# leighghunt/kart

Measured on AMD Instinct MI355X. Metric: feature deltas classified+field-diffed/sec (M/s) at 1/2/4/8 GPUs; % HBM peak, higher is better.
Workload: dtype u8/u64 (integer + fp64 compare); 1 GPU; C3: ONE 100000000-polygon int-PK layer, 10% edits (4% geometry + 4% attribute updates, 1% del, 1% ins), two-commit diff + field diff; features=100000000, delta_order=walk (= key) order, then pk order (kd_delta_pk_order), side_order=git tree (walk) order as listed, no side sort, parallelism=bucket-range shards x1

## Files before the change

### kart_amd/csrc/kd_classify.hip

```cpp
#include <cstdlib>

#include "kd_join.h"

namespace kd {

#ifndef KD_RS3_PROBE_NOSEARCH
#define KD_RS3_PROBE_NOSEARCH 0
#endif
#ifndef KD_RS3_PROBE_NOOID
#define KD_RS3_PROBE_NOOID 0
#endif
#ifndef KD_RS3_PROBE_NONAMES
#define KD_RS3_PROBE_NONAMES 0
#endif
constexpr int C3_NT = 256;
constexpr int C3_CH = 1024;
#ifndef KD_C3_SAMPLE_BITS
#define KD_C3_SAMPLE_BITS 11
#endif
constexpr int C3_SAMPLE_BITS = KD_C3_SAMPLE_BITS;
constexpr int C3_SAMPLES = 1 << C3_SAMPLE_BITS;

struct Resolve3Args {
    const u64 *A, *O, *T;
// ... 232 lines not shown
        if (tid == 0) {
            if (tclean) atomicAdd((unsigned long long*)g.counts, (unsigned long long)tclean);
            if (base + cnt == n) {
                g.counts[1] = exc + tc;
                g.counts[2] = exm + tm;
            }
        }
        u64 pc = exc + (off & 0xFFFF), pm = exm + (off >> 16);
#pragma unroll
        for (int j = 0; j < PT; j++) {
            if (cls[j] == 2) {
                u32* o = g.out_conf + 3 * pc;
                o[0] = ia[j]; o[1] = io[j]; o[2] = itt[j];
                pc++;
            } else if (cls[j] == 1) {
                g.out_md[pm] = rec[j];
                pm++;
            }
        }
    }
}

}

using namespace kd;

int kd::resolve3_have_a(kd_ctx* ctx, const kd_side& A, const kd_side& O, const kd_side& T, const u32* cand3,
                        const u64* c2, u32* d_conf, uint2* d_md, u64* counts, u32* derr, const u32* pA, const u32* pO,
                        const u32* pT) {
    const bool perm = pA || pO || pT;
    int rc;
    const u64 nA = A.n, nO = O.n, nT = T.n;
    const u64 nchunk = (nO + nT) / C3_CH + 2;
    void *desc, *aux, *dz;
    if ((rc = ensure(ctx, "c3.desc", 2 * nchunk * 8, &desc))) return rc;
    const bool fresh_aux = ctx->bufs["c3.aux"].p == nullptr;
    if ((rc = ensure(ctx, "c3.aux", 64, &aux))) return rc;
    if (fresh_aux) KD_HIP(hipMemsetAsync(aux, 0, 64, ctx->stream));
    if ((rc = device_zeros(ctx, &dz))) return rc;
    rc = launch(ctx, "k_sorted3", [&] {
        const u64 blocks = std::min<u64>((2 * nchunk + 255) / 256, (u64)ctx->n_cu * 8);
        hipLaunchKernelGGL(k_sorted3, dim3((unsigned)std::max<u64>(blocks, 1)), dim3(256), 0, ctx->stream,
                           (const u64*)dz, (u64)0, (u64*)desc, 2 * nchunk, (u32*)aux, counts);
    });
    if (rc) return rc;
    const int occ_r3a = occupancy(ctx, perm ? (const void*)k_resolve3<C3_NT, true, true> : (const void*)k_resolve3<C3_NT, false, true>,
                                  C3_NT, 0);
    auto ptr = [&](const void* p, u64 n) { return n && p ? p : (const void*)dz; };
    Resolve3Args g{};
    g.A = (const u64*)dz; g.O = (const u64*)ptr(O.key, nO); g.T = (const u64*)ptr(T.key, nT);
    g.oA = (const u32*)ptr(A.oid, nA); g.oO = (const u32*)ptr(O.oid, nO); g.oT = (const u32*)ptr(T.oid, nT);
    g.nA = nA; g.nO = nO;
    g.nmA = (const u8*)ptr(A.name, nA); g.nmO = (const u8*)ptr(O.name, nO); g.nmT = (const u8*)ptr(T.name, nT);
    g.noA = (const u64*)ptr(A.name_off, nA); g.noO = (const u64*)ptr(O.name_off, nO); g.noT = (const u64*)ptr(T.name_off, nT);
    g.hash_mode = A.key_mode == KD_KEY_HASH;
    g.cand = nullptr; g.cand3 = cand3; g.c2 = c2;
    g.pA = (const u32*)ptr(pA, nA); g.pO = (const u32*)ptr(pO, nO); g.pT = (const u32*)ptr(pT, nT);
    g.desc = (u64*)desc; g.nchunk = nchunk; g.aux = (u32*)aux;
    g.out_conf = d_conf; g.out_md = d_md; g.counts = counts; g.err = derr;
    const u64 grid = std::min<u64>((nO + nT) / C3_CH + 1, (u64)ctx->n_cu * (u64)occ_r3a);
    return launch(ctx, "k_resolve3", [&] {
        if (perm) hipLaunchKernelGGL((k_resolve3<C3_NT, true, true>), dim3((unsigned)grid), dim3(C3_NT), 0, ctx->stream, g);
        else hipLaunchKernelGGL((k_resolve3<C3_NT, false, true>), dim3((unsigned)grid), dim3(C3_NT), 0, ctx->stream, g);
    });
}

int kd::stage_side(kd_ctx* ctx, const kd_side* s, const char* tag, kd_side* dev) {
    *dev = *s;
    dev->mem = KD_MEM_DEVICE;
    std::string p(tag);
    int rc;
    if ((rc = stage_in(ctx, (p + ".key").c_str(), s->key, s->n * 8, s->mem, (const void**)&dev->key))) return rc;
    if ((rc = stage_in(ctx, (p + ".oid").c_str(), s->oid, s->n * 20, s->mem, (const void**)&dev->oid))) return rc;
    if (s->key_mode == KD_KEY_HASH && s->n) {
        KD_CHECK(s->name_off && s->name, "KD_KEY_HASH side without filenames");
        u64 nbytes = s->mem == KD_MEM_HOST ? s->name_off[s->n] : 0;
        if (s->mem == KD_MEM_DEVICE) {
            KD_HIP(hipMemcpy(&nbytes, s->name_off + s->n, 8, hipMemcpyDeviceToHost));
        }
        if ((rc = stage_in(ctx, (p + ".noff").c_str(), s->name_off, (s->n + 1) * 8, s->mem, (const void**)&dev->name_off))) return rc;
        if ((rc = stage_in(ctx, (p + ".name").c_str(), s->name, nbytes ? nbytes : 1, s->mem, (const void**)&dev->name))) return rc;
    }
    return KD_OK;
}

int kd::check_side(const kd_side* s, const char* which) {
    KD_CHECK(s, "%s side is NULL", which);
    KD_CHECK(s->n == 0 || (s->key && s->oid), "%s side: key/oid NULL", which);
    KD_CHECK(s->mem == KD_MEM_HOST || s->mem == KD_MEM_DEVICE, "%s side: bad mem", which);
    KD_CHECK(s->key_mode == KD_KEY_INT || s->key_mode == KD_KEY_HASH, "%s side: bad key_mode", which);
    return KD_OK;
}

static int merge3_device(kd_ctx* ctx, const kd_side& A, const kd_side& O, const kd_side& T, u32* d_conf, uint2* d_md,
                         u64* counts, u32* derr, const u32* pA = nullptr, const u32* pO = nullptr,
                         const u32* pT = nullptr) {
    const bool perm = pA || pO || pT;
    int rc;
    const u64 nA = A.n, nO = O.n, nT = T.n;
    if (nO + nT > 0 && ctx->opt.merge3_join)
        return merge3_join_device(ctx, A, O, T, d_conf, d_md, counts, derr, pA, pO, pT);
    const u64 nchunk = (nO + nT) / C3_CH + 2;
    void *cand, *c2, *desc, *aux, *dz;
    if ((rc = ensure(ctx, "c3.cand", (nO + nT + 1) * 8, &cand))) return rc;
    if ((rc = ensure(ctx, "c3.c2", 64, &c2))) return rc;
    if ((rc = ensure(ctx, "c3.desc", 2 * nchunk * 8, &desc))) return rc;
    const bool fresh_aux = ctx->bufs["c3.aux"].p == nullptr;
    if ((rc = ensure(ctx, "c3.aux", 64, &aux))) return rc;
    if (fresh_aux) KD_HIP(hipMemsetAsync(aux, 0, 64, ctx->stream));
    if ((rc = device_zeros(ctx, &dz))) return rc;
    const u64* kA = nA ? A.key : (const u64*)dz;
    rc = launch(ctx, "k_sorted3", [&] {
        const u64 work = std::max<u64>(nA / 2, 2 * nchunk);
        const u64 blocks = std::min<u64>((work + 255) / 256, (u64)ctx->n_cu * 8);
        hipLaunchKernelGGL(k_sorted3, dim3((unsigned)std::max<u64>(blocks, 1)), dim3(256), 0, ctx->stream, kA, nA,
                           (u64*)desc, 2 * nchunk, (u32*)aux, counts);
    });
    if (rc) return rc;
    if ((rc = diff2_device(ctx, &O, &T, 0, (u32*)cand, nullptr, (u64*)c2, derr, perm ? pO : nullptr,
                           perm ? pT : nullptr)))
        return rc;
    ctx->occ_resolve3 = occupancy(ctx, perm ? (const void*)k_resolve3<C3_NT, true, false> : (const void*)k_resolve3<C3_NT, false, false>,
                                  C3_NT, 0);
    auto ptr = [&](const void* p, u64 n) { return n && p ? p : (const void*)dz; };
    Resolve3Args g;
    g.A = kA; g.O = (const u64*)ptr(O.key, nO); g.T = (const u64*)ptr(T.key, nT);
    g.oA = (const u32*)ptr(A.oid, nA); g.oO = (const u32*)ptr(O.oid, nO); g.oT = (const u32*)ptr(T.oid, nT);
    g.nA = nA; g.nO = nO;
    g.nmA = (const u8*)ptr(A.name, nA); g.nmO = (const u8*)ptr(O.name, nO); g.nmT = (const u8*)ptr(T.name, nT);
    g.noA = (const u64*)ptr(A.name_off, nA); g.noO = (const u64*)ptr(O.name_off, nO); g.noT = (const u64*)ptr(T.name_off, nT);
    g.hash_mode = A.key_mode == KD_KEY_HASH;
    g.cand = (const uint2*)cand; g.c2 = (const u64*)c2;
    g.pA = (const u32*)ptr(pA, nA); g.pO = (const u32*)ptr(pO, nO); g.pT = (const u32*)ptr(pT, nT);
    g.desc = (u64*)desc; g.nchunk = nchunk; g.aux = (u32*)aux;
    g.out_conf = d_conf; g.out_md = d_md; g.counts = counts; g.err = derr;
    const u64 grid = std::min<u64>((nO + nT) / C3_CH + 1, (u64)ctx->n_cu * (u64)ctx->occ_resolve3);
    return launch(ctx, "k_resolve3", [&] {
        if (perm) hipLaunchKernelGGL((k_resolve3<C3_NT, true, false>), dim3((unsigned)grid), dim3(C3_NT), 0, ctx->stream, g);
        else hipLaunchKernelGGL((k_resolve3<C3_NT, false, false>), dim3((unsigned)grid), dim3(C3_NT), 0, ctx->stream, g);
    });
}

extern "C" {

int kd_reserve(kd_ctx* ctx, uint64_t max_entries_per_side, uint64_t max_updates) {
    KD_CHECK(ctx, "kd_reserve: ctx NULL");
    KD_HIP(hipSetDevice(ctx->device));
    u64 total = 2 * max_entries_per_side;
    u64 ntiles = (total + C2_TILE - 1) / C2_TILE + 1;
    void* p;
    int rc;
    if ((rc = ensure(ctx, "c2.part", (ntiles + 1) * 8, &p))) return rc;
    if ((rc = ensure(ctx, "c2.tcnt", ntiles * 16, &p))) return rc;
    if ((rc = ensure(ctx, "c2.gsum", 2 * (ntiles / 64 + 1) * 8, &p))) return rc;
    if ((rc = ensure(ctx, "c2.sdel", ntiles * (C2_TILE + 64) * 8, &p))) return rc;
    (void)max_updates;
    return KD_OK;
}

int kd_diff2_device(kd_ctx* ctx, const kd_side* base, const kd_side* target, uint32_t flags, uint32_t* d_delta,
                    uint32_t* d_upd, uint64_t* d_counts, uint32_t* d_err) {
    KD_CHECK(ctx, "kd_diff2_device: ctx NULL");
    int rc;
    if ((rc = check_side(base, "base")) || (rc = check_side(target, "target"))) return rc;
    KD_CHECK(base->mem == KD_MEM_DEVICE && target->mem == KD_MEM_DEVICE, "kd_diff2_device: sides must be device memory");
    KD_CHECK(d_delta && d_counts && d_err, "kd_diff2_device: NULL output");
    KD_HIP(hipSetDevice(ctx->device));
    return diff2_device(ctx, base, target, flags, d_delta, d_upd, d_counts, d_err);
}

int kd_diff2_device_perm(kd_ctx* ctx, const kd_side* base, const kd_side* target, const uint32_t* base_order,
                         const uint32_t* target_order, uint32_t flags, uint32_t* d_delta, uint32_t* d_upd,
                         uint64_t* d_counts, uint32_t* d_err) {
    KD_CHECK(ctx, "kd_diff2_device_perm: ctx NULL");
    int rc;
    if ((rc = check_side(base, "base")) || (rc = check_side(target, "target"))) return rc;
    KD_CHECK(base->mem == KD_MEM_DEVICE && target->mem == KD_MEM_DEVICE, "kd_diff2_device_perm: sides must be device memory");
    KD_CHECK(d_delta && d_counts && d_err, "kd_diff2_device_perm: NULL output");
    KD_CHECK((base->n == 0 || base_order) && (target->n == 0 || target_order), "kd_diff2_device_perm: NULL order");
    KD_HIP(hipSetDevice(ctx->device));
    return diff2_device(ctx, base, target, flags, d_delta, d_upd, d_counts, d_err,
                        base_order ? base_order : (const u32*)nullptr, target_order);
}

int kd_diff2_device_ex(kd_ctx* ctx, const kd_side* base, const kd_side* target, const uint32_t* base_order,
                       const uint32_t* target_order, uint32_t flags, uint32_t* d_delta, uint32_t* d_upd,
                       uint64_t* d_delta_key, uint64_t* d_upd_key, uint64_t* d_counts, uint32_t* d_err) {
    KD_CHECK(ctx, "kd_diff2_device_ex: ctx NULL");
    int rc;
    if ((rc = check_side(base, "base")) || (rc = check_side(target, "target"))) return rc;
    KD_CHECK(base->mem == KD_MEM_DEVICE && target->mem == KD_MEM_DEVICE, "kd_diff2_device_ex: sides must be device memory");
    KD_CHECK(d_delta && d_counts && d_err, "kd_diff2_device_ex: NULL output");
    KD_CHECK(!base_order == !target_order, "kd_diff2_device_ex: both orders or neither");
    KD_CHECK(!d_upd_key || (d_upd && d_delta_key), "kd_diff2_device_ex: update keys need the update list and delta keys");
    KD_HIP(hipSetDevice(ctx->device));
    void* dz = nullptr;
    if (base_order && (rc = device_zeros(ctx, &dz))) return rc;
    const u32* oa = base_order ? (base->n ? base_order : (const u32*)dz) : nullptr;
    const u32* ob = target_order ? (target->n ? target_order : (const u32*)dz) : nullptr;
    return diff2_device(ctx, base, target, flags, d_delta, d_upd, d_counts, d_err, oa, ob, d_delta_key, d_upd_key);
}

int kd_diff2_step(kd_ctx* ctx, const kd_step* s) {
    KD_CHECK(ctx && s, "kd_diff2_step: NULL");
    int rc;
    if ((rc = check_side(s->base, "base")) || (rc = check_side(s->target, "target"))) return rc;
    KD_CHECK(s->base->mem == KD_MEM_DEVICE && s->target->mem == KD_MEM_DEVICE, "kd_diff2_step: sides must be device memory");
    KD_CHECK(s->d_delta && s->d_counts && s->d_err, "kd_diff2_step: NULL output");
    KD_CHECK(!s->base_order == !s->target_order, "kd_diff2_step: both orders or neither");
    KD_CHECK(!s->d_upd_key || (s->d_upd && s->d_delta_key), "kd_diff2_step: update keys need the update list and delta keys");
    const bool have_fd = s->old_blobs != nullptr;
    KD_CHECK(!have_fd || (s->new_blobs && s->maps && s->d_masks && s->d_status), "kd_diff2_step: field diff: NULL argument");
    const bool have_dpk = s->d_delta_pk != nullptr, have_upk = s->d_upd_pk != nullptr;
    KD_CHECK(!have_dpk || s->d_delta_perm, "kd_diff2_step: d_delta_pk without d_delta_perm");
    KD_CHECK(!have_upk || (s->d_upd_perm && s->d_upd), "kd_diff2_step: d_upd_pk needs d_upd_perm and the update list");
    KD_HIP(hipSetDevice(ctx->device));
    void* dz = nullptr;
    if ((rc = device_zeros(ctx, &dz))) return rc;
    const u32* oa = s->base_order ? (s->base->n ? s->base_order : (const u32*)dz) : nullptr;
    const u32* ob = s->target_order ? (s->target->n ? s->target_order : (const u32*)dz) : nullptr;
    Diff2Place pl;
    if ((rc = diff2_front(ctx, s->base, s->target, s->flags, s->d_delta, s->d_upd, s->d_counts, s->d_err, oa, ob,
                          s->d_delta_key, s->d_upd_key, &pl)))
        return rc;
    const int ov = ctx->opt.step_overlap;
    auto field_diff = [&]() -> int {
        return have_fd ? kd_fielddiff(ctx, s->old_blobs, s->new_blobs, s->d_pairs, s->upd_cap, s->d_counts + 1,
                                      KD_MEM_DEVICE, s->maps, s->d_masks, s->d_status, KD_MEM_DEVICE)
                       : KD_OK;
    };
    auto pk_orders = [&](bool lds_free) -> int {
        int r = KD_OK;
        if (have_dpk)
            r = delta_pk_order(ctx, s->base, s->target, s->d_delta, s->d_delta_key, s->delta_cap, s->d_counts + 3,
                               s->pk_lo, s->pk_hi, s->d_delta_pk, s->d_delta_perm, lds_free);
        if (!r && have_upk)
            r = delta_pk_order(ctx, s->base, s->target, s->d_upd, s->d_upd_key, s->upd_cap, s->d_counts + 1, s->pk_lo,
                               s->pk_hi, s->d_upd_pk, s->d_upd_perm, lds_free);
        return r;
    };
    const bool place_aside = !(have_fd && s->d_pairs);
    const bool overlap = ov > 0 && have_fd && pl.needed && (place_aside || have_dpk || have_upk) &&
                         s->base->n + s->target->n >= ctx->opt.step_overlap_min;
    const int wave = ctx->opt.pkm_wave;
    if (!overlap) {
        if ((rc = diff2_place(ctx, pl)) || (rc = field_diff())) return rc;
        return pk_orders(wave > 0);
    }
    if (!ctx->side_stream) {
        KD_HIP(hipStreamCreateWithFlags(&ctx->side_stream, hipStreamNonBlocking));
        KD_HIP(hipEventCreateWithFlags(&ctx->ev_fork, hipEventDisableTiming));
        KD_HIP(hipEventCreateWithFlags(&ctx->ev_join, hipEventDisableTiming));
    }
    const hipStream_t main = ctx->stream, side = ctx->side_stream;
    if (!place_aside && (rc = diff2_place(ctx, pl))) return rc;
    KD_HIP(hipEventRecord(ctx->ev_fork, main));
    auto side_work = [&]() -> int {
        StreamScope scope(ctx, side);
        KD_HIP(hipStreamWaitEvent(side, ctx->ev_fork, 0));
        int r = place_aside ? diff2_place(ctx, pl) : KD_OK;
        return r ? r : pk_orders(wave != 0);
    };
    int rc_fd, rc_side = KD_OK;
    if (ov == 2) {
        rc_side = side_work();
        rc_fd = field_diff();
    } else {
        rc_fd = field_diff();
        if (!rc_fd) rc_side = side_work();
    }
    hipError_t e = hipEventRecord(ctx->ev_join, side);
    if (e == hipSuccess) e = hipStreamWaitEvent(main, ctx->ev_join, 0);
    if (e != hipSuccess) {
        const hipError_t e2 = hipStreamSynchronize(side);
        if (!rc_fd && !rc_side) {
            set_error("kd_diff2_step: join: %s", hipGetErrorString(e2 != hipSuccess ? e2 : e));
            return KD_EHIP;
        }
    }
    return rc_fd ? rc_fd : rc_side;
}

int kd_diff2(kd_ctx* ctx, const kd_side* base, const kd_side* target, uint32_t flags, kd_diff_result** out) {
    KD_CHECK(ctx && out, "kd_diff2: NULL");
    int rc;
    if ((rc = check_side(base, "base")) || (rc = check_side(target, "target"))) return rc;
    KD_HIP(hipSetDevice(ctx->device));
    host_mark(ctx, nullptr);
    kd_side A, B;
    if ((rc = stage_side(ctx, base, "in.a", &A)) || (rc = stage_side(ctx, target, "in.b", &B))) return rc;
    host_mark(ctx, "kd_diff2 stage");
    u64 total = base->n + target->n;
    void *dd, *du, *dc;
    if ((rc = ensure(ctx, "out.delta", (total + 1) * 8, &dd))) return rc;
    if ((rc = ensure(ctx, "out.upd", (total + 1) * 8, &du))) return rc;
    if ((rc = ensure(ctx, "out.counts", 64, &dc))) return rc;
    host_mark(ctx, "kd_diff2 ensure");
    u64* counts = (u64*)dc;
    u32* derr = (u32*)(counts + 4);
    if ((rc = diff2_device(ctx, &A, &B, flags, (u32*)dd, (u32*)du, counts, derr))) return rc;
    host_mark(ctx, "kd_diff2 kernels");
    u64 hc[5];
    KD_HIP(hipMemcpyAsync(hc, dc, 40, hipMemcpyDeviceToHost, ctx->stream));
    KD_HIP(hipStreamSynchronize(ctx->stream));
    u32 err = (u32)(hc[4] & 0xFFFFFFFFu);
    if (err) {
        set_error("kd_diff2: %s", (err & 1) ? "side keys not strictly ascending" : "hash key collision between different filenames");
        return KD_EUNSUPPORTED;
    }
    u64 nd = hc[3], nu = hc[1];
    host_mark(ctx, "kd_diff2 counts");
    size_t bytes = sizeof(kd_diff_result) + (nd + nu) * 8 + 16;
    kd_diff_result* r = (kd_diff_result*)std::malloc(bytes);
    KD_CHECK(r, "kd_diff2: out of host memory");
    host_mark(ctx, "kd_diff2 malloc");
    r->n_insert = hc[0]; r->n_update = hc[1]; r->n_delete = hc[2]; r->n_delta = nd;
    r->delta = (u32*)(r + 1);
    r->upd = r->delta + 2 * nd;
    if (nd) {
        if ((rc = stage_d2h(ctx, r->delta, dd, nd * 8)) || (nu && (rc = stage_d2h(ctx, r->upd, du, nu * 8)))) {
            std::free(r);
            return rc;
        }
    }
    host_mark(ctx, "kd_diff2 results");
    prof_flush(ctx);
    *out = r;
    return KD_OK;
}

int kd_merge3(kd_ctx* ctx, const kd_side* anc, const kd_side* ours, const kd_side* theirs, uint32_t flags,
              kd_merge_result** out) {
    (void)flags;
    KD_CHECK(ctx && out, "kd_merge3: NULL");
    int rc;
    if ((rc = check_side(anc, "ancestor")) || (rc = check_side(ours, "ours")) || (rc = check_side(theirs, "theirs"))) return rc;
    KD_CHECK(anc->key_mode == ours->key_mode && ours->key_mode == theirs->key_mode, "kd_merge3: key modes differ");
    KD_CHECK(anc->n < 0xFFFFFFFFull && ours->n < 0xFFFFFFFFull && theirs->n < 0xFFFFFFFFull, "kd_merge3: side too large");
    KD_HIP(hipSetDevice(ctx->device));
    kd_side A, O, T;
    if ((rc = stage_side(ctx, anc, "in.a", &A)) || (rc = stage_side(ctx, ours, "in.b", &O)) ||
        (rc = stage_side(ctx, theirs, "in.c", &T)))
        return rc;
    const u64 nA = A.n, nO = O.n, nT = T.n;
    void *oc, *om, *dc;
    if ((rc = ensure(ctx, "c3.oc", (nA + nO + nT + 1) * 12, &oc))) return rc;
    if ((rc = ensure(ctx, "c3.om", (nO + nT + 1) * 8, &om))) return rc;
    if ((rc = ensure(ctx, "c3.counts", 64, &dc))) return rc;
    u64* counts = (u64*)dc;
    u32* derr = (u32*)(counts + 4);
    if ((rc = merge3_device(ctx, A, O, T, (u32*)oc, (uint2*)om, counts, derr))) return rc;
    u64 hc[5];
    KD_HIP(hipMemcpyAsync(hc, dc, 40, hipMemcpyDeviceToHost, ctx->stream));
    KD_HIP(hipStreamSynchronize(ctx->stream));
    u32 err = (u32)(hc[4] & 0xFFFFFFFFu);
    if (err) {
        set_error("kd_merge3: err=0x%x (%s)", err,
                  (err & 1) ? "keys not strictly ascending" : (err & 2) ? "hash key collision" : "tile overflow");
        return KD_EUNSUPPORTED;
    }
    u64 nc = hc[1], nm = hc[2];
    kd_merge_result* r = (kd_merge_result*)std::malloc(sizeof(kd_merge_result) + nc * 12 + nm * 8 + 16);
    KD_CHECK(r, "kd_merge3: out of host memory");
    r->n_clean = hc[0]; r->n_conflict = nc; r->n_mdelta = nm;
    r->conflict = (u32*)(r + 1);
    r->mdelta = r->conflict + 3 * nc;
    if ((nc && (rc = stage_d2h(ctx, r->conflict, oc, nc * 12))) || (nm && (rc = stage_d2h(ctx, r->mdelta, om, nm * 8)))) {
        std::free(r);
        return rc;
    }
    prof_flush(ctx);
    *out = r;
    return KD_OK;
}

int kd_merge3_device(kd_ctx* ctx, const kd_side* anc, const kd_side* ours, const kd_side* theirs, uint32_t flags,
                     uint32_t* d_conflict, uint32_t* d_mdelta, uint64_t* d_counts, uint32_t* d_err) {
    (void)flags;
    KD_CHECK(ctx && d_conflict && d_mdelta && d_counts && d_err, "kd_merge3_device: NULL");
    int rc;
    if ((rc = check_side(anc, "ancestor")) || (rc = check_side(ours, "ours")) || (rc = check_side(theirs, "theirs"))) return rc;
    KD_CHECK(anc->mem == KD_MEM_DEVICE && ours->mem == KD_MEM_DEVICE && theirs->mem == KD_MEM_DEVICE,
             "kd_merge3_device: sides must be device memory");
    KD_CHECK(anc->key_mode == ours->key_mode && ours->key_mode == theirs->key_mode, "kd_merge3_device: key modes differ");
    KD_CHECK(anc->n < 0xFFFFFFFFull && ours->n < 0xFFFFFFFFull && theirs->n < 0xFFFFFFFFull,
             "kd_merge3_device: side too large");
    KD_HIP(hipSetDevice(ctx->device));
    return merge3_device(ctx, *anc, *ours, *theirs, d_conflict, (uint2*)d_mdelta, d_counts, d_err);
}

int kd_merge3_device_perm(kd_ctx* ctx, const kd_side* anc, const kd_side* ours, const kd_side* theirs,
                          const uint32_t* anc_order, const uint32_t* ours_order, const uint32_t* theirs_order,
                          uint32_t flags, uint32_t* d_conflict, uint32_t* d_mdelta, uint64_t* d_counts, uint32_t* d_err) {
    (void)flags;
    KD_CHECK(ctx && d_conflict && d_mdelta && d_counts && d_err, "kd_merge3_device_perm: NULL");
    int rc;
    if ((rc = check_side(anc, "ancestor")) || (rc = check_side(ours, "ours")) || (rc = check_side(theirs, "theirs"))) return rc;
    KD_CHECK(anc->mem == KD_MEM_DEVICE && ours->mem == KD_MEM_DEVICE && theirs->mem == KD_MEM_DEVICE,
             "kd_merge3_device_perm: sides must be device memory");
    KD_CHECK(anc->key_mode == ours->key_mode && ours->key_mode == theirs->key_mode, "kd_merge3_device_perm: key modes differ");
    KD_CHECK(anc->n < 0xFFFFFFFFull && ours->n < 0xFFFFFFFFull && theirs->n < 0xFFFFFFFFull,
             "kd_merge3_device_perm: side too large");
    KD_CHECK((anc->n == 0 || anc_order) && (ours->n == 0 || ours_order) && (theirs->n == 0 || theirs_order),
             "kd_merge3_device_perm: NULL order");
    KD_HIP(hipSetDevice(ctx->device));
    void* dz;
    if ((rc = device_zeros(ctx, &dz))) return rc;
    auto ord = [&](const uint32_t* p) { return p ? p : (const u32*)dz; };
    return merge3_device(ctx, *anc, *ours, *theirs, d_conflict, (uint2*)d_mdelta, d_counts, d_err, ord(anc_order),
                         ord(ours_order), ord(theirs_order));
}

}
// ... 1 lines not shown
```

### kart_amd/csrc/kd_classify2.hip

```cpp
#include <cstdlib>

#include "kd_join.h"

namespace kd {

constexpr u64 C2_GROUP = 64;
#ifndef KD_C2_STAGE_PAD
#define KD_C2_STAGE_PAD 32
#endif
constexpr u64 C2_STAGE = C2_TILE + KD_C2_STAGE_PAD;
#ifndef KD_J2_NAME_HALO
#define KD_J2_NAME_HALO 64
#endif
constexpr u64 J2_NAME_HALO = KD_J2_NAME_HALO;
#ifndef KD_PLACE_NT
#define KD_PLACE_NT 64
#endif


template <int PW>
__device__ __forceinline__ u64 mp_search(const u64* __restrict__ A, const u64* __restrict__ B, u64 d, u64 lo, u64 hi) {
    const int lane = threadIdx.x & 63, sub = lane % PW, grp = lane / PW;
    while (hi > lo) {
        const u64 step = (hi - lo + PW - 1) / PW;
        const u64 probe = lo + step * (u64)(sub + 1) - 1;
        bool p = true;
        if (probe < hi) p = A[probe] > B[d - 1 - probe];
        const unsigned long long bal = (__ballot(p) >> (grp * PW)) & ((PW == 64) ? ~0ull : ((1ull << PW) - 1));
        if (bal == 0) return hi;
        const int f = __ffsll(bal) - 1;
        const u64 nh = lo + step * (u64)(f + 1) - 1;
        lo = lo + step * (u64)f;
        hi = nh < hi ? nh : hi;
        if (step == 1) return hi;
    }
    return lo;
}

template <int PW>
__device__ __forceinline__ u64 mp_search_guided(const u64* __restrict__ A, const u64* __restrict__ B, u64 d, u64 lo,
                                                u64 hi, u64 guess, u64 step) {
    if (hi <= lo) return lo;
    const int lane = threadIdx.x & 63, sub = lane % PW, grp = lane / PW;
    const u64 span = step * (PW / 2);
    const u64 g0 = guess > lo + span ? guess - span : lo;
    u64 probe = g0 + step * (u64)sub;
    if (probe > hi) probe = hi;
    bool p = true;
    if (probe < hi) p = A[probe] > B[d - 1 - probe];
    const unsigned long long bal = (__ballot(p) >> (grp * PW)) & ((PW == 64) ? ~0ull : ((1ull << PW) - 1));
    const int f = bal ? __ffsll(bal) - 1 : PW;
    const u64 pf = f < PW ? (g0 + step * (u64)f < hi ? g0 + step * (u64)f : hi) : hi;
    const u64 pl = f > 0 ? (g0 + step * (u64)(f - 1) < hi ? g0 + step * (u64)(f - 1) : hi) : lo;
    const u64 nlo = f > 0 ? pl + 1 : lo, nhi = pf;
    return mp_search<PW>(A, B, d, nlo < nhi ? nlo : nhi, nhi);
}

#ifndef KD_PTOP
#define KD_PTOP 16
#endif
constexpr int C2_PG = 32, C2_PNT = 256;
template <int TILE>
__global__ __launch_bounds__(C2_PNT) void k_partition2(const u64* __restrict__ A, u64 nA, const u64* __restrict__ B,
                                                       u64 nB, u64 ntiles, u64* __restrict__ part,
                                                       u64* __restrict__ zero_counts, u32* __restrict__ zero_err,
                                                       u64* __restrict__ zero_buf, u64 n_zero) {
    if (blockIdx.x == 0 && threadIdx.x < 4) zero_counts[threadIdx.x] = 0;
    if (blockIdx.x == 0 && threadIdx.x == 4) *zero_err = 0;
    for (u64 k = (u64)blockIdx.x * C2_PNT + threadIdx.x; k < n_zero; k += (u64)gridDim.x * C2_PNT) zero_buf[k] = 0;
    __shared__ u64 s_end[2];
    const int tid = threadIdx.x;
    const u64 total = nA + nB;
    const u64 t0 = (u64)blockIdx.x * C2_PG, t1 = t0 + C2_PG < ntiles ? t0 + C2_PG : ntiles;
    if (tid < 2 * KD_PTOP) {
        const u64 t = tid < KD_PTOP ? t0 : t1;
        u64 d = t * (u64)TILE;
        if (d > total) d = total;
        const u64 guess = (u64)((double)d * (double)nA / (double)(total ? total : 1));
        const u64 i = mp_search_guided<KD_PTOP>(A, B, d, d > nB ? d - nB : 0, d < nA ? d : nA, guess, 2048 / KD_PTOP);
        if ((tid & (KD_PTOP - 1)) == 0) s_end[tid / KD_PTOP] = i;
    }
    __syncthreads();
    const u64 i0 = s_end[0], i1 = s_end[1];
    const u64 d0 = t0 * (u64)TILE, d1 = t1 * (u64)TILE < total ? t1 * (u64)TILE : total;
    const u64 j0 = d0 - i0, j1 = d1 - i1;
    if (tid == 0) part[t0] = i0;
    if (tid == 1 && t1 == ntiles) part[ntiles] = i1;
    const u64 t = t0 + 1 + (u64)(tid / 8);
    if (t < t1) {
        const u64 d = t * (u64)TILE;
        const u64 lo = (d > j1 && d - j1 > i0) ? d - j1 : i0, hi = i1 < d - j0 ? i1 : d - j0;
        const u64 guess = d1 > d0 ? i0 + (u64)((double)(d - d0) * (double)(i1 - i0) / (double)(d1 - d0)) : lo;
        const u64 i = mp_search_guided<8>(A, B, d, lo, hi, guess, 16);
        if ((tid & 7) == 0) part[t] = i;
    }
}

struct Join2Args {
    const u64* A;
    const u8* oidA;
    u64 nA;
    const u64* B;
    const u8* oidB;
    u64 nB;
    const u64* part;
    const u8* nameA;
    const u64* nameOffA;
    const u8* nameB;
    const u64* nameOffB;
    int hash_mode;
    const u8* dummy;
    const u32* ordA;
    const u32* ordB;
    uint2* stage_delta;
    u32* tile_cnt;
    u64* gsum;
    uint2* out_delta;
    uint2* out_upd;
    u64* stage_dkey;
    u64* out_dkey;
    u64* out_ukey;
    u64* counts;
    u32* err;
    u64 ntiles;
    int walk;
};

struct Range {
    u64 base;
    u32 nch;
    u32 skew;
};

__device__ __forceinline__ Range mk_range(const void* p, u64 first_byte, u64 end_byte) {
    Range r;
    const u64 a0 = (u64)p + first_byte, a1 = (u64)p + end_byte;
    r.base = a0 & ~(u64)15;
    r.skew = (u32)(a0 - r.base);
    r.nch = end_byte > first_byte ? (u32)((a1 - r.base + 15) >> 4) : 0;
    return r;
}

template <int NT, int IPT>
struct Join2Lds {
    static constexpr int TILE = NT * IPT;
    static constexpr int CHK = (8 * (TILE + 1) + 16 + 15) / 16 + 4;
#ifndef KD_J2_NAME_CH
#define KD_J2_NAME_CH 1900
#endif
    static constexpr int NMCH = KD_J2_NAME_CH;
    static constexpr int OCH = (20 * (TILE + 1) + 32 + 15) / 16 + 4;
    static constexpr int rounds(int w) { return w <= 0 ? 0 : 1 + rounds((w + 3) / 4 - 1); }
    static constexpr int SEARCH_ROUNDS = rounds(TILE);
};

typedef __attribute__((address_space(3))) void* lds_vp;
typedef const __attribute__((address_space(1))) void* glb_vp;

struct TileGeo {
    u64 i0, i1, j0, j1, j1e, lbA, lbB;
    int na, nb;
    bool ok, has_lbA, has_lbB, has_la;
};

__device__ __forceinline__ u64 uni64(u64 x) {
    return (u64)(u32)__builtin_amdgcn_readfirstlane((u32)x) | (u64)(u32)__builtin_amdgcn_readfirstlane((u32)(x >> 32)) << 32;
}

__device__ __forceinline__ TileGeo tile_geo_from(const Join2Args& g, u64 t, int TILE, u64 p0, u64 p1) {
    TileGeo q;
    const u64 total = g.nA + g.nB;
    const u64 d0 = t * (u64)TILE, d1 = d0 + TILE < total ? d0 + TILE : total;
    q.i0 = uni64(p0);
    q.i1 = uni64(p1);
    q.ok = !(q.i1 < q.i0 || d1 - q.i1 < d0 - q.i0 || q.i1 - q.i0 > d1 - d0);
    if (!q.ok) q.i1 = q.i0 = d0 < g.nA ? d0 : g.nA;
    q.j0 = d0 - q.i0;
    q.j1 = q.ok ? d1 - q.i1 : q.j0;
    if (q.j1 > g.nB) q.j1 = q.j0 = g.nB;
    q.j1e = q.j1 < g.nB ? q.j1 + 1 : q.j1;
    q.na = (int)(q.i1 - q.i0);
    q.nb = (int)(q.j1 - q.j0);
    q.has_lbA = q.i0 > 0;
    q.has_lbB = q.j0 > 0;
    q.has_la = q.j1 < g.nB;
    q.lbA = q.lbB = 0;
    return q;
}

__device__ __forceinline__ TileGeo tile_geo(const Join2Args& g, u64 t, int TILE) {
    return tile_geo_from(g, t, TILE, g.part[t], g.part[t + 1]);
}

struct TileRanges {
    Range ka, kb;
    u32 c1;
};

__device__ __forceinline__ TileRanges tile_ranges(const Join2Args& g, const TileGeo& q) {
    TileRanges r;
    r.ka = mk_range(g.A, 8 * (q.i0 - q.has_lbA), 8 * q.i1);
    r.kb = mk_range(g.B, 8 * (q.j0 - q.has_lbB), 8 * q.j1e);
    r.c1 = r.ka.nch;
    return r;
}

enum : u32 { R_NONE = 0, R_DEL = 1, R_MATCH = 2, R_INS = 3 };

#ifndef KD_J2_PROBE
#define KD_J2_PROBE 0
#endif

constexpr int J2_GW = 8;
constexpr int split_rounds_for(int w) {
    return w <= 0 ? 0 : 1 + split_rounds_for(((w + 3) / 4 - 1 > w - 3 * ((w + 3) / 4)) ? (w + 3) / 4 - 1 : w - 3 * ((w + 3) / 4));
}
static_assert(split_rounds_for(2 * J2_GW - 1) == 2, "the bracket is meant to be finished in 2 rounds");

template <int ROUNDS>
__device__ __forceinline__ void split_rounds(const u64* sA, const u64* sB, int dd, int& lo, int& hi) {
#pragma unroll
    for (int r = 0; r < ROUNDS; r++) {
        const int w = hi - lo;
        const int s = (w + 3) >> 2;
        const int p1 = lo + s - 1, p2 = p1 + s, p3 = p2 + s;
        const int hm = w > 0 ? hi - 1 : lo;
        const int q1 = p1 > lo ? p1 : lo, q2 = p2 < hm ? p2 : hm, q3 = p3 < hm ? p3 : hm;
        const u64 a1 = sA[q1], v1 = sB[dd - 1 - q1], a2 = sA[q2], v2 = sB[dd - 1 - q2];
        const u64 a3 = sA[q3], v3 = sB[dd - 1 - q3];
        const bool b1 = a1 > v1;
        const bool b2 = (p2 >= hi) | (a2 > v2);
        const bool b3 = (p3 >= hi) | (a3 > v3);
        const int m2 = p2 < hi ? p2 : hi, m3 = p3 < hi ? p3 : hi;
        int nlo = p3 + 1, nhi = hi;
        nlo = b3 ? p2 + 1 : nlo;
        nhi = b3 ? m3 : nhi;
        nlo = b2 ? p1 + 1 : nlo;
        nhi = b2 ? m2 : nhi;
        nlo = b1 ? lo : nlo;
        nhi = b1 ? p1 : nhi;
        lo = w > 0 ? nlo : lo;
        hi = w > 0 ? nhi : hi;
    }
}

template <int IPT>
__device__ __forceinline__ void walk_items_full(const u64* sA, const u64* sB, const TileGeo& q, int ia0, int dd,
                                                u32 rec[IPT], bool& bad) {
    const int na = q.na, nb = q.nb;
    const int nbx = nb + (q.has_la ? 1 : 0);
    int ia = ia0, jb = dd - ia0;
    const int amax = na > 0 ? na - 1 : 0, bmax = nbx > 0 ? nbx - 1 : 0;
    u64 ka = sA[ia < amax ? ia : amax], kb = sB[jb < bmax ? jb : bmax];
    bool ap_ok = (ia > 0) | q.has_lbA, bp_ok = (jb > 0) | q.has_lbB;
    u64 ap = sA[ia - 1], bp = sB[jb - 1];
    u32 b = 0;
#pragma unroll
    for (int k = 0; k < IPT; k++) {
        const bool ta = (jb >= nb) | ((ia < na) & (ka <= kb));
        const bool m = (jb < nbx) & (kb == ka);
        const bool partner = ap_ok & (ap == kb);
        const u32 kt = R_DEL + (u32)m, kf = partner ? (u32)R_NONE : (u32)R_INS;
        rec[k] = ((ta ? kt : kf) << 25) | ((u32)jb << 12) | (u32)ia;
        b |= (u32)(ap_ok & (ap >= ka)) & (u32)ta;
        b |= (u32)(bp_ok & (bp >= kb)) & (u32)!ta;
        ap = ta ? ka : ap;
        bp = ta ? bp : kb;
        ap_ok |= ta;
        bp_ok |= !ta;
// ... 77 lines not shown
    else walk_items<IPT>(sA, sB, q, lo, dd, cnt, rec, bad);
#endif
}

template <int IPT>
__device__ __forceinline__ void range_keys(const u64* s, int n, u64 k[IPT + 1]) {
    const int x0 = (int)threadIdx.x * IPT - 1, last = n > 0 ? n - 1 : 0;
#pragma unroll
    for (int j = 0; j <= IPT; j++) k[j] = s[x0 + j < last ? x0 + j : last];
}

template <int IPT>
__device__ __forceinline__ bool keys_unsorted(const u64 k[IPT + 1], int n, bool has_lb) {
    const int x0 = (int)threadIdx.x * IPT - 1;
    bool bad = false;
#pragma unroll
    for (int j = 1; j <= IPT; j++) bad |= (x0 + j < n) & ((x0 + j > 0) | has_lb) & (k[j - 1] >= k[j]);
    return bad;
}

template <int IPT, bool PERM>
__device__ __forceinline__ void tile_rows(const Join2Args& g, const TileGeo& q, const u32 rec[IPT], u32 ra[IPT],
                                          u32 rb[IPT]) {
    typedef const __attribute__((address_space(1))) u32* gp32;
#pragma unroll
    for (int k = 0; k < IPT; k++) {
        ra[k] = (u32)q.i0 + (rec[k] & 0xFFF);
        rb[k] = (u32)q.j0 + ((rec[k] >> 12) & 0xFFF);
    }
    if (PERM) {
#pragma unroll
        for (int k = 0; k < IPT; k++) {
            const bool m = (rec[k] >> 25) == R_MATCH;
            const gp32 oa = m ? (gp32)(g.ordA + ra[k]) : (gp32)g.dummy;
            const gp32 ob = m ? (gp32)(g.ordB + rb[k]) : (gp32)g.dummy;
            ra[k] = *oa;
            rb[k] = *ob;
        }
    }
}

template <int IPT>
__device__ __forceinline__ void tile_oid_cmp(const Join2Args& g, u32 rec[IPT], const u32 ra[IPT], const u32 rb[IPT]) {
    typedef const __attribute__((address_space(1))) u32* gp32;
    u32 x[IPT][5], y[IPT][5];
#pragma unroll
    for (int k = 0; k < IPT; k++) {
        const bool m = (rec[k] >> 25) == R_MATCH;
        const gp32 pa = m ? (gp32)(g.oidA + 20ull * ra[k]) : (gp32)g.dummy;
        const gp32 pb = m ? (gp32)(g.oidB + 20ull * rb[k]) : (gp32)g.dummy;
#pragma unroll
        for (int w = 0; w < 5; w++) { x[k][w] = pa[w]; y[k][w] = pb[w]; }
    }
#pragma unroll
    for (int k = 0; k < IPT; k++) {
        u32 d = 0;
#pragma unroll
        for (int w = 0; w < 5; w++) d |= x[k][w] ^ y[k][w];
        if ((rec[k] >> 25) == R_MATCH && d) rec[k] |= 1u << 24;
    }
}

template <int IPT, bool PERM>
__device__ __forceinline__ void tile_oid_global(const Join2Args& g, const TileGeo& q, u32 rec[IPT], u32 ra[IPT],
                                                u32 rb[IPT]) {
    tile_rows<IPT, PERM>(g, q, rec, ra, rb);
    tile_oid_cmp<IPT>(g, rec, ra, rb);
}

template <int IPT>
__device__ __forceinline__ void tile_names(const Join2Args& g, const u32 rec[IPT], const u32 ia[IPT], const u32 jb[IPT]) {
    u32 act = 0;
#pragma unroll
    for (int k = 0; k < IPT; k++) act |= (u32)((rec[k] >> 25) == R_MATCH) << k;
    if (names_ne_batch<IPT, 8>(g.nameA, g.nameOffA, ia, g.nameB, g.nameOffB, jb, act)) atomicOr(g.err, 2u);
}

struct TileCounts {
    u32 fd, fu;
    u32 od, ou;
    u32 tnd, tnu, tdel;
};

__device__ __forceinline__ void lds_barrier() {
    __builtin_amdgcn_s_waitcnt(0xC07F);
    __builtin_amdgcn_s_barrier();
}

template <int NT, int IPT, bool LB = false>
__device__ __forceinline__ TileCounts tile_counts(const u32 rec[IPT], u32* s_wave) {
    TileCounts c;
    const int tid = threadIdx.x, lane = tid & 63, wid = tid >> 6;
    u32 fd = 0, fu = 0, fx = 0;
#pragma unroll
    for (int k = 0; k < IPT; k++) {
        const u32 kind = rec[k] >> 25, chg = (rec[k] >> 24) & 1;
        const u32 isx = (u32)(kind == R_DEL), isi = (u32)(kind == R_INS), isu = (u32)(kind == R_MATCH) & chg;
        fd |= (isx | isi | isu) << k;
        fu |= isu << k;
        fx |= isx << k;
    }
    u32 od = 0, ou = 0, wd = 0, wu = 0, wx = 0;
#pragma unroll
    for (int k = 0; k < IPT; k++) {
        const u64 bd = __ballot((fd >> k) & 1);
        const u64 bu = __ballot((fu >> k) & 1);
        const u64 bx = __ballot((fx >> k) & 1);
        od += __builtin_amdgcn_mbcnt_hi((u32)(bd >> 32), __builtin_amdgcn_mbcnt_lo((u32)bd, 0));
        ou += __builtin_amdgcn_mbcnt_hi((u32)(bu >> 32), __builtin_amdgcn_mbcnt_lo((u32)bu, 0));
        wd += __popcll(bd);
        wu += __popcll(bu);
        wx += __popcll(bx);
    }
    if (lane == 0) { s_wave[wid] = wd; s_wave[NT / 64 + wid] = wu; s_wave[2 * NT / 64 + wid] = wx; }
    if (LB) lds_barrier();
    else __syncthreads();
    u32 tnd = 0, tnu = 0, tdel = 0;
#pragma unroll
    for (int w = 0; w < NT / 64; w++) {
        const u32 a = s_wave[w], b = s_wave[NT / 64 + w];
        if (w < wid) { od += a; ou += b; }
        tnd += a;
        tnu += b;
        tdel += s_wave[2 * NT / 64 + w];
    }
    c.fd = fd; c.fu = fu; c.od = od; c.ou = ou; c.tnd = tnd; c.tnu = tnu; c.tdel = tdel;
    return c;
}

template <int IPT>
__device__ __forceinline__ void tile_write(const u32 rec[IPT], const TileCounts& c, u64 i0, u64 j0,
                                           uint2* __restrict__ sd, uint2* __restrict__ su, const u64* sA, const u64* sB,
                                           u64* __restrict__ kd, u64* __restrict__ ku) {
    u32 od = c.od, ou = c.ou;
    const u32 has_su = su != nullptr;
    const bool keys = kd != nullptr;
#pragma unroll
    for (int k = 0; k < IPT; k++) {
        const u32 kind = rec[k] >> 25, ia = rec[k] & 0xFFF, jb = (rec[k] >> 12) & 0xFFF;
        const u32 isd = (c.fd >> k) & 1, isu = (c.fu >> k) & 1;
        const uint2 v = make_uint2(kind == R_INS ? KD_NONE : (u32)(i0 + ia), kind == R_DEL ? KD_NONE : (u32)(j0 + jb));
        if (isd) sd[od] = v;
        if (keys && isd) {
            const u64 key = kind == R_INS ? sB[jb] : sA[ia];
            kd[od] = key;
            if ((isu & has_su) && ku) ku[ou] = key;
        }
        od += isd;
        if (isu & has_su) su[ou] = v;
        ou += isu;
    }
}

template <int NT, int IPT, bool UNORD, bool HASH, bool PERM, bool OL = false>
__global__ __launch_bounds__(NT) void k_join2(Join2Args g) {
    using LD = Join2Lds<NT, IPT>;
    static_assert(LD::TILE <= 4095, "per-item records hold 12-bit local indices");
    constexpr bool LNAMES = HASH;
    constexpr bool LOIDS = OL && !HASH && !PERM;
    __shared__ u32x4 s_ch[LD::CHK];
    __shared__ u32x4 s_nm[LNAMES ? LD::NMCH : 1];
    __shared__ u32x4 s_oid[LOIDS ? LD::OCH : 1];
    __shared__ u32 s_wave[3 * NT / 64];
    __shared__ u64 s_base[2];
    const int tid = threadIdx.x;
    const u64 tile = blockIdx.x;
    const TileGeo q = tile_geo(g, tile, LD::TILE);
    if (!q.ok && tid == 0) atomicOr(g.err, 1u);
    const TileRanges r = tile_ranges(g, q);
    u64 nmA0 = 0, nmA1 = 0, nmB0 = 0, nmB1 = 0;
    const u64 rA0 = PERM ? (q.i0 > J2_NAME_HALO ? q.i0 - J2_NAME_HALO : 0) : q.i0;
    const u64 rA1 = PERM ? min(q.i1 + J2_NAME_HALO, g.nA) : q.i1;
    const u64 rB0 = PERM ? (q.j0 > J2_NAME_HALO ? q.j0 - J2_NAME_HALO : 0) : q.j0;
    const u64 rB1 = PERM ? min(q.j1e + J2_NAME_HALO, g.nB) : q.j1e;
    if (LNAMES) {
        nmA0 = g.nameOffA[rA0]; nmA1 = g.nameOffA[rA1];
        nmB0 = g.nameOffB[rB0]; nmB1 = g.nameOffB[rB1];
    }
    auto dma2 = [&](const Range& R0, const Range& R1, u32 c1, u32x4* dst) {
        constexpr int NW = NT / 64;
        const int wid = __builtin_amdgcn_readfirstlane(tid >> 6), lane = tid & 63;
        u32 q0 = 0;
#pragma unroll
        for (int k = 0; k < 2; k++) {
            const Range& R = k == 0 ? R0 : R1;
            const u32 off = k == 0 ? 0 : c1;
            const u32 np = (R.nch + 63) >> 6;
            for (u32 p = (u32)(wid + NW - (int)(q0 % NW)) % NW; p < np; p += NW) {
                const u32 c = 64 * p + lane;
                if (c < R.nch)
                    __builtin_amdgcn_global_load_lds((glb_vp)(R.base + 16ull * c), (lds_vp)(dst + off + 64 * p), 16, 0, 0);
            }
            q0 += np;
        }
    };
    dma2(r.ka, r.kb, r.c1, s_ch);
    Range roA{}, roB{};
    if (LOIDS) {
        roA = mk_range(g.oidA, 20 * q.i0, 20 * q.i1);
        roB = mk_range(g.oidB, 20 * q.j0, 20 * q.j1e);
        dma2(roA, roB, roA.nch, s_oid);
    }
    __syncthreads();
    Range rnA{}, rnB{};
    bool lnames = false;
    if (LNAMES) {
        nmA0 = uni64(nmA0); nmA1 = uni64(nmA1); nmB0 = uni64(nmB0); nmB1 = uni64(nmB1);
        rnA = mk_range(g.nameA, nmA0, nmA1);
        rnB = mk_range(g.nameB, nmB0, nmB1);
        lnames = nmA1 >= nmA0 && nmB1 >= nmB0 && (u64)rnA.nch + rnB.nch <= (u64)LD::NMCH;
        if (lnames) dma2(rnA, rnB, rnA.nch, s_nm);
    }
    const u64* sA = (const u64*)((const u8*)s_ch + r.ka.skew) + q.has_lbA;
    const u64* sB = (const u64*)((const u8*)(s_ch + r.c1) + r.kb.skew) + q.has_lbB;
    u32 rec[IPT];
    bool bad = false;
    const bool walk1 = g.walk != 0;
    const bool check1 = walk1 && !(KD_J2_PROBE & 2);
    u64 ca[IPT + 1], cb[IPT + 1];
    if (check1) { range_keys<IPT>(sA, q.na, ca); range_keys<IPT>(sB, q.nb, cb); }
    tile_walk<NT, IPT>(sA, sB, q, walk1, rec, bad);
    if (check1) {
        bad |= keys_unsorted<IPT>(ca, q.na, q.has_lbA);
        bad |= keys_unsorted<IPT>(cb, q.nb, q.has_lbB);
    }
    if (!walk1 && !(KD_J2_PROBE & 2)) {
        for (int x = tid; x < q.na; x += NT) bad |= (x > 0 || q.has_lbA) && sA[x - 1] >= sA[x];
        for (int x = tid; x < q.nb; x += NT) bad |= (x > 0 || q.has_lbB) && sB[x - 1] >= sB[x];
    }
    u32 ra[IPT], rb[IPT];
    u32 oa0[IPT], oa1[IPT], ob0[IPT], ob1[IPT];
    if (!LOIDS) tile_rows<IPT, PERM>(g, q, rec, ra, rb);
    if (LNAMES && lnames) {
        const u32* offA = (const u32*)g.nameOffA;
        const u32* offB = (const u32*)g.nameOffB;
#pragma unroll
        for (int k = 0; k < IPT; k++) {
            const bool m = (rec[k] >> 25) == R_MATCH;
            const u64 i = m ? ra[k] : 0, j = m ? rb[k] : 0;
            oa0[k] = m ? offA[2 * i] : 0u; oa1[k] = m ? offA[2 * i + 2] : 0u;
            ob0[k] = m ? offB[2 * j] : 0u; ob1[k] = m ? offB[2 * j + 2] : 0u;
        }
    }
    if (LOIDS) {
        typedef const __attribute__((address_space(3))) u32* l32;
        const u32 ob = (u32)(size_t)(const __attribute__((address_space(3))) u32x4*)s_oid;
        const u32 baseA = ob + roA.skew, baseB = ob + 16 * roA.nch + roB.skew;
#pragma unroll
        for (int k = 0; k < IPT && !(KD_J2_PROBE & 4); k++) {
            const bool m = (rec[k] >> 25) == R_MATCH;
            const u32 pa = baseA + 20 * (m ? (rec[k] & 0xFFF) : 0), pb = baseB + 20 * (m ? ((rec[k] >> 12) & 0xFFF) : 0);
            u32 d = 0;
#pragma unroll
            for (int w = 0; w < 5; w++) d |= *(l32)(size_t)(pa + 4 * w) ^ *(l32)(size_t)(pb + 4 * w);
            if (m && d) rec[k] |= 1u << 24;
        }
    } else {
        tile_oid_cmp<IPT>(g, rec, ra, rb);
    }
    if (LNAMES && lnames) {
        __syncthreads();
        const u32 nm = (u32)(size_t)(const __attribute__((address_space(3))) u32x4*)s_nm;
        const u32 baseA = nm + rnA.skew, baseB = nm + 16 * rnA.nch + rnB.skew;
        bool ne = false;
#pragma unroll
        for (int k = 0; k < IPT; k++) {
            if ((rec[k] >> 25) != R_MATCH) continue;
            const u32 la = oa1[k] - oa0[k], lb = ob1[k] - ob0[k];
            if (PERM && (ra[k] < rA0 || ra[k] >= rA1 || rb[k] < rB0 || rb[k] >= rB1))
                ne |= !names_eq(g.nameA, g.nameOffA, ra[k], g.nameB, g.nameOffB, rb[k]);
            else
                ne |= la != lb || !lds_eq_bytes(baseA + (oa0[k] - (u32)nmA0), baseB + (ob0[k] - (u32)nmB0), la);
        }
        if (ne) atomicOr(g.err, 2u);
    } else if (HASH) {
        tile_names<IPT>(g, rec, ra, rb);
    }
    if (bad) atomicOr(g.err, 1u);
    const TileCounts c = tile_counts<NT, IPT>(rec, s_wave);
    uint2 *sd, *su = nullptr;
    u64 *kd, *ku = nullptr;
    if (UNORD) {
        if (tid < 4) {
            const u64 v = tid == 0 ? c.tnd : tid == 1 ? c.tnu : tid == 2 ? c.tnd - c.tnu - c.tdel : c.tdel;
            const int slot = tid == 0 ? 3 : tid == 1 ? 1 : tid == 2 ? 0 : 2;
            const u64 old = v ? atomicAdd((unsigned long long*)(g.counts + slot), (unsigned long long)v) : 0;
            if (tid < 2) s_base[tid] = old;
        }
        __syncthreads();
        sd = g.out_delta + s_base[0];
        su = g.out_upd ? g.out_upd + s_base[1] : nullptr;
        kd = g.out_dkey ? g.out_dkey + s_base[0] : nullptr;
        ku = g.out_dkey && g.out_upd && g.out_ukey ? g.out_ukey + s_base[1] : nullptr;
    } else {
        sd = g.stage_delta + tile * (u64)C2_STAGE;
        kd = g.stage_dkey ? g.stage_dkey + tile * (u64)C2_STAGE : nullptr;
    }
    tile_write<IPT>(rec, c, q.i0, q.j0, sd, su, sA, sB, kd, ku);
    if (!UNORD && tid == 0) {
        u32* cc = g.tile_cnt + 4 * tile;
        const u32 tins = c.tnd - c.tnu - c.tdel;
        cc[0] = tins;
        cc[1] = c.tnu;
        cc[2] = c.tdel;
        cc[3] = c.tnd;
        u64* gs = g.gsum + 2 * (tile / C2_GROUP);
        atomicAdd((unsigned long long*)gs, (unsigned long long)(c.tnd | (u64)c.tnu << 32));
        atomicAdd((unsigned long long*)gs + 1, (unsigned long long)(tins | (u64)c.tdel << 32));
    }
}

template <int NT, int IPT>
struct J2RTile {
    TileGeo q;
    TileRanges r;
    Range oa, ob;
    u32 n0, n1, n2, n3;
};

template <int NT, int IPT>
__device__ __forceinline__ void j2r_plan(const Join2Args& g, u64 tile, u64 p0, u64 p1, J2RTile<NT, IPT>& T) {
    using LD = Join2Lds<NT, IPT>;
    T.q = tile_geo_from(g, tile, LD::TILE, p0, p1);
    T.r = tile_ranges(g, T.q);
    T.oa = mk_range(g.oidA, 20 * T.q.i0, 20 * T.q.i1);
    T.ob = mk_range(g.oidB, 20 * T.q.j0, 20 * T.q.j1e);
    T.n0 = T.r.ka.nch;
    T.n1 = T.n0 + T.r.kb.nch;
    T.n2 = T.n1 + T.oa.nch;
    T.n3 = T.n2 + T.ob.nch;
}

template <int NT, int IPT>
__global__ __launch_bounds__(NT) void k_join2r(Join2Args g) {
    using LD = Join2Lds<NT, IPT>;
    static_assert(LD::TILE <= 4095, "per-item records hold 12-bit local indices");
    constexpr int P = (LD::CHK + LD::OCH + NT - 1) / NT;
    __shared__ u32x4 s_ch[LD::CHK];
    __shared__ u32x4 s_oid[LD::OCH];
    __shared__ u32 s_wave[3 * NT / 64];
    typedef __attribute__((address_space(3))) u32x4* l128;
    typedef const __attribute__((address_space(1))) u32x4* g128;
    const int tid = threadIdx.x;
    const u64 ntiles = g.ntiles;
    u64 tile = blockIdx.x;
    if (tile >= ntiles) return;
    J2RTile<NT, IPT> cur, nxt;
    u32x4 buf[P];
    auto fetch = [&](const J2RTile<NT, IPT>& T) {
#pragma unroll
        for (int p = 0; p < P; p++) {
            const u32 c = tid + NT * p;
            u64 src = 0;
            if (c < T.n0) src = T.r.ka.base + 16ull * c;
            else if (c < T.n1) src = T.r.kb.base + 16ull * (c - T.n0);
            else if (c < T.n2) src = T.oa.base + 16ull * (c - T.n1);
            else if (c < T.n3) src = T.ob.base + 16ull * (c - T.n2);
            if (c < T.n3) buf[p] = *(g128)src;
        }
    };
    auto deposit = [&](const J2RTile<NT, IPT>& T) {
#pragma unroll
        for (int p = 0; p < P; p++) {
            const u32 c = tid + NT * p;
            if (c < T.n0) *(l128)(s_ch + c) = buf[p];
            else if (c < T.n1) *(l128)(s_ch + T.r.c1 + (c - T.n0)) = buf[p];
            else if (c < T.n2) *(l128)(s_oid + (c - T.n1)) = buf[p];
            else if (c < T.n3) *(l128)(s_oid + T.oa.nch + (c - T.n2)) = buf[p];
        }
    };
    j2r_plan<NT, IPT>(g, tile, g.part[tile], g.part[tile + 1], cur);
    fetch(cur);
    deposit(cur);
    u64 nt = tile + gridDim.x;
    u64 np0 = 0, np1 = 0;
    if (nt < ntiles) { np0 = g.part[nt]; np1 = g.part[nt + 1]; }
    lds_barrier();
    for (;;) {
        const bool more = nt < ntiles;
        if (more) {
            j2r_plan<NT, IPT>(g, nt, np0, np1, nxt);
            fetch(nxt);
        }
        const u64 nn = nt + gridDim.x;
        u64 ap0 = 0, ap1 = 0;
        if (more && nn < ntiles) { ap0 = g.part[nn]; ap1 = g.part[nn + 1]; }
        const TileGeo& q = cur.q;
        if (!q.ok && tid == 0) atomicOr(g.err, 1u);
        const u64* sA = (const u64*)((const u8*)s_ch + cur.r.ka.skew) + q.has_lbA;
        const u64* sB = (const u64*)((const u8*)(s_ch + cur.r.c1) + cur.r.kb.skew) + q.has_lbB;
        u32 rec[IPT];
        bool bad = false;
        tile_walk<NT, IPT>(sA, sB, q, g.walk != 0, rec, bad);
        for (int x = tid; x < q.na; x += NT) bad |= (x > 0 || q.has_lbA) && sA[x - 1] >= sA[x];
        for (int x = tid; x < q.nb; x += NT) bad |= (x > 0 || q.has_lbB) && sB[x - 1] >= sB[x];
        {
            typedef const __attribute__((address_space(3))) u32* l32;
            const u32 ob = (u32)(size_t)(const __attribute__((address_space(3))) u32x4*)s_oid;
            const u32 baseA = ob + cur.oa.skew, baseB = ob + 16 * cur.oa.nch + cur.ob.skew;
#pragma unroll
            for (int k = 0; k < IPT; k++) {
                const bool m = (rec[k] >> 25) == R_MATCH;
                const u32 pa = baseA + 20 * (m ? (rec[k] & 0xFFF) : 0), pb = baseB + 20 * (m ? ((rec[k] >> 12) & 0xFFF) : 0);
                u32 d = 0;
#pragma unroll
                for (int w = 0; w < 5; w++) d |= *(l32)(size_t)(pa + 4 * w) ^ *(l32)(size_t)(pb + 4 * w);
                if (m && d) rec[k] |= 1u << 24;
            }
        }
        if (bad) atomicOr(g.err, 1u);
        const TileCounts c = tile_counts<NT, IPT, true>(rec, s_wave);
        uint2* sd = g.stage_delta + tile * (u64)C2_STAGE;
        u64* kd = g.stage_dkey ? g.stage_dkey + tile * (u64)C2_STAGE : nullptr;
        tile_write<IPT>(rec, c, q.i0, q.j0, sd, nullptr, sA, sB, kd, nullptr);
        if (tid == 0) {
            u32* cc = g.tile_cnt + 4 * tile;
            const u32 tins = c.tnd - c.tnu - c.tdel;
            cc[0] = tins;
            cc[1] = c.tnu;
            cc[2] = c.tdel;
            cc[3] = c.tnd;
            u64* gs = g.gsum + 2 * (tile / C2_GROUP);
            atomicAdd((unsigned long long*)gs, (unsigned long long)(c.tnd | (u64)c.tnu << 32));
            atomicAdd((unsigned long long*)gs + 1, (unsigned long long)(tins | (u64)c.tdel << 32));
        }
        if (!more) break;
        lds_barrier();
        deposit(nxt);
        lds_barrier();
        cur = nxt;
        tile = nt;
        nt = nn;
        np0 = ap0;
        np1 = ap1;
    }
}

constexpr int GSCAN_GPT = 8;
__global__ __launch_bounds__(1024) void k_gscan2(const u64* __restrict__ gsum, u64 ngroups, u64* __restrict__ gpre,
                                                 u64* __restrict__ counts, int layout) {
    __shared__ u64 s_w[4][16];
    const int tid = threadIdx.x, lane = tid & 63, wid = tid >> 6;
    const u32x4* g4 = (const u32x4*)gsum;
    u32x4* p4 = (u32x4*)gpre;
    u64 cd = 0, cu = 0, ci = 0, cx = 0;
    for (u64 base = 0; base < ngroups; base += 1024 * GSCAN_GPT) {
        const u64 k0 = base + (u64)tid * GSCAN_GPT;
        u32x4 v[GSCAN_GPT];
#pragma unroll
        for (int j = 0; j < GSCAN_GPT; j++) v[j] = k0 + j < ngroups ? g4[k0 + j] : u32x4{0u, 0u, 0u, 0u};
        u64 td = 0, tu = 0, ti = 0, tx = 0;
#pragma unroll
        for (int j = 0; j < GSCAN_GPT; j++) {
            td += v[j].x; tu += v[j].y; ti += v[j].z; tx += v[j].w;
        }
        u64 sd = td, su = tu, si = ti, sx = tx;
#pragma unroll
        for (int o = 1; o < 64; o <<= 1) {
            const u64 yd = __shfl_up(sd, o, 64), yu = __shfl_up(su, o, 64);
            if (lane >= o) { sd += yd; su += yu; }
        }
#pragma unroll
        for (int o = 32; o > 0; o >>= 1) { si += __shfl_xor(si, o, 64); sx += __shfl_xor(sx, o, 64); }
        if (lane == 63) { s_w[0][wid] = sd; s_w[1][wid] = su; }
        if (lane == 0) { s_w[2][wid] = si; s_w[3][wid] = sx; }
        __syncthreads();
        u64 wd = 0, wu = 0, Td = 0, Tu = 0, Ti = 0, Tx = 0;
#pragma unroll
        for (int w = 0; w < 16; w++) {
            if (w < wid) { wd += s_w[0][w]; wu += s_w[1][w]; }
            Td += s_w[0][w]; Tu += s_w[1][w]; Ti += s_w[2][w]; Tx += s_w[3][w];
        }
        u64 pd = cd + wd + sd - td, pu = cu + wu + su - tu;
#pragma unroll
        for (int j = 0; j < GSCAN_GPT; j++) {
            if (k0 + j < ngroups) p4[k0 + j] = u32x4{(u32)pd, (u32)(pd >> 32), (u32)pu, (u32)(pu >> 32)};
            pd += v[j].x;
            pu += v[j].y;
        }
        cd += Td; cu += Tu; ci += Ti; cx += Tx;
        __syncthreads();
    }
    if (tid == 0) {
        counts[0] = ci;
        counts[1] = layout ? cd : cu;
        counts[2] = layout ? cu : cx;
        counts[3] = layout ? 0 : cd;
    }
}

template <int NT>
__global__ __launch_bounds__(NT) void k_place2(const uint2* __restrict__ stage_delta, const u32* __restrict__ tile_cnt,
                                               const u64* __restrict__ gpre, int tile_items,
                                               uint2* __restrict__ out_delta, uint2* __restrict__ out_upd,
                                               const u64* __restrict__ stage_dkey, u64* __restrict__ out_dkey,
                                               u64* __restrict__ out_ukey) {
    static_assert(NT == 64, "k_place2: one wave per tile");
    const int tid = threadIdx.x;
    const u64 t = blockIdx.x;
    const u64 grp = t / C2_GROUP;
    const u64 t_lo = grp * C2_GROUP;
    const uint2* sdp = stage_delta + t * (u64)tile_items;
    const uint2 v0 = sdp[tid];
    const u64* skd = out_dkey ? stage_dkey + t * (u64)tile_items : nullptr;
    const u64 kd0 = skd ? skd[tid] : 0;
    u64 pd = 0, pu = 0;
    if (tid < (int)(t - t_lo)) {
        const uint4 c = *(const uint4*)(tile_cnt + 4 * (t_lo + tid));
        pd = c.w;
        pu = c.y;
    }
    const u64 gd = gpre[2 * grp], gu = gpre[2 * grp + 1];
    const uint4 ownc = *(const uint4*)(tile_cnt + 4 * t);
#pragma unroll
    for (int o = 32; o > 0; o >>= 1) { pd += __shfl_xor(pd, o, 64); pu += __shfl_xor(pu, o, 64); }
    pd += gd;
    pu += gu;
    const u32 nd = (u32)__builtin_amdgcn_readfirstlane((int)ownc.w);
    const bool ukeys = out_dkey && out_upd && out_ukey;
    u32 urun = 0;
    auto emit = [&](u32 r, const uint2 v, const u64 k) {
        const bool ok = r < nd;
        const bool isu = ok && v.x != KD_NONE && v.y != KD_NONE;
        const u64 bu = __ballot(isu);
        const u32 ur = urun + __builtin_amdgcn_mbcnt_hi((u32)(bu >> 32), __builtin_amdgcn_mbcnt_lo((u32)bu, 0));
        urun += (u32)__popcll(bu);
        if (ok) out_delta[pd + r] = v;
        if (isu && out_upd) out_upd[pu + ur] = v;
        if (ok && out_dkey) out_dkey[pd + r] = k;
        if (isu && ukeys) out_ukey[pu + ur] = k;
    };
    emit((u32)tid, v0, kd0);
    for (u32 r0 = NT; r0 < nd; r0 += 4 * NT) {
        uint2 v[4];
        u64 kk[4];
#pragma unroll
        for (int j = 0; j < 4; j++) {
            const u32 r = r0 + j * NT + tid;
            v[j] = make_uint2(KD_NONE, KD_NONE);
            kk[j] = 0;
            if (r < nd) {
                v[j] = sdp[r];
                if (skd) kk[j] = skd[r];
            }
        }
#pragma unroll
        for (int j = 0; j < 4; j++) emit(r0 + j * NT + tid, v[j], kk[j]);
    }
}


struct Join3Args {
    Join2Args j;
    const u64* K;
    const u8* oidK;
    const u8* nameK;
    const u64* nameOffK;
    const u32* ordK;
    u64 nK;
    const u64* apart;
    u32* stage_conf;
    uint2* stage_md;
    const u64* nsplit;
};
#ifndef KD_J3_ACAP
#define KD_J3_ACAP 1024
#endif
constexpr int J3_ACAP = KD_J3_ACAP;
#ifndef KD_J3_IPT
#define KD_J3_IPT 3
#endif
constexpr int J3_IPT = KD_J3_IPT;
constexpr int J3_TILE = C2_NT * J3_IPT;
#ifndef KD_J3_NAME_CH
#define KD_J3_NAME_CH 1425
#endif

template <int PW>
__device__ __forceinline__ u64 lb_search(const u64* __restrict__ K, u64 key, u64 lo, u64 hi) {
    const int lane = threadIdx.x & 63, sub = lane % PW, grp = lane / PW;
    while (hi > lo) {
        const u64 step = (hi - lo + PW - 1) / PW;
        const u64 probe = lo + step * (u64)(sub + 1) - 1;
        bool p = true;
        if (probe < hi) p = K[probe] >= key;
        const unsigned long long bal = (__ballot(p) >> (grp * PW)) & ((PW == 64) ? ~0ull : ((1ull << PW) - 1));
        if (bal == 0) return hi;
        const int f = __ffsll(bal) - 1;
        const u64 nh = lo + step * (u64)(f + 1) - 1;
        lo = lo + step * (u64)f;
        hi = nh < hi ? nh : hi;
        if (step == 1) return hi;
    }
    return lo;
}

template <int PW>
__device__ __forceinline__ u64 lb_guided(const u64* __restrict__ K, u64 n, u64 key, u64 guess, u64 step) {
    const int lane = threadIdx.x & 63, sub = lane % PW, grp = lane / PW;
    const u64 span = step * (PW / 2);
    const u64 g0 = guess > span ? guess - span : 0;
    u64 probe = g0 + step * (u64)sub;
    if (probe > n) probe = n;
    const bool p = probe >= n || K[probe] >= key;
    const unsigned long long bal = (__ballot(p) >> (grp * PW)) & ((PW == 64) ? ~0ull : ((1ull << PW) - 1));
    const int f = bal ? __ffsll(bal) - 1 : PW;
    const u64 pf = f < PW ? (g0 + step * (u64)f < n ? g0 + step * (u64)f : n) : n;
    const u64 pl = f > 0 ? (g0 + step * (u64)(f - 1) < n ? g0 + step * (u64)(f - 1) : n) : 0;
    const u64 nlo = f > 0 ? pl + 1 : 0;
    return lb_search<PW>(K, key, nlo < pf ? nlo : pf, pf);
}

__global__ __launch_bounds__(256) void k_apart3(const u64* __restrict__ O, u64 nO, const u64* __restrict__ T, u64 nT,
                                                const u64* __restrict__ part, u64 ntiles, int tile_items,
                                                const u64* __restrict__ K, u64 nK, u64* __restrict__ apart) {
    const u64 t = ((u64)blockIdx.x * 256 + threadIdx.x) / 8;
    if (t > ntiles) return;
    u64 r;
    if (t == 0) r = 0;
    else if (t == ntiles) r = nK;
    else {
        const u64 i = part[t], d = t * (u64)tile_items, j = d - i;
        const u64 a = i < nO ? O[i] : ~0ull, b = j < nT ? T[j] : ~0ull;
        const u64 key = a < b ? a : b;
        const u64 guess = nO ? (u64)((double)i / (double)nO * (double)nK) : (u64)((double)d / (double)(nO + nT) * (double)nK);
        r = lb_guided<8>(K, nK, key, guess < nK ? guess : nK, 256);
    }
    if ((threadIdx.x & 7) == 0) apart[t] = r;
}

template <int NT>
__device__ __forceinline__ u32 dma_range(const Range& R, u32x4* dst, u32 q0) {
    constexpr int NW = NT / 64;
    const int wid = __builtin_amdgcn_readfirstlane(threadIdx.x >> 6), lane = threadIdx.x & 63;
    const u32 np = (R.nch + 63) >> 6;
    for (u32 p = (u32)(wid + NW - (int)(q0 % NW)) % NW; p < np; p += NW) {
        const u32 c = 64 * p + lane;
        if (c < R.nch) __builtin_amdgcn_global_load_lds((glb_vp)(R.base + 16ull * c), (lds_vp)(dst + 64 * p), 16, 0, 0);
    }
    return q0 + np;
// ... 579 lines not shown
        } else {
        u32 rk3 = ik, ro = io, rt = itt;
        if (PERM) {
            rk3 = ik != KD_NONE ? (lk ? sOrdK[lo] : *(gp32)(g3.ordK + ik)) : KD_NONE;
            ro = io != KD_NONE ? sOrdO[ia] : KD_NONE;
            rt = itt != KD_NONE ? sOrdT[jb] : KD_NONE;
        }
        const gp32 pk = rk3 != KD_NONE ? (gp32)(g3.oidK + 20ull * rk3) : (gp32)g.dummy;
        const gp32 po = ro != KD_NONE ? (gp32)(g.oidA + 20ull * ro) : (gp32)g.dummy;
        const gp32 pt = rt != KD_NONE ? (gp32)(g.oidB + 20ull * rt) : (gp32)g.dummy;
        const bool chk = HASH && ik != KD_NONE && (io != KD_NONE || itt != KD_NONE);
        const bool side_o = io != KD_NONE;
        const u32 srow = side_o ? ro : rt;
        u64 kn0 = 0, kn1 = 0, sn0 = 0, sn1 = 0;
        if (HASH) {
            const u64* offS = side_o ? g.nameOffA : g.nameOffB;
            kn0 = g3.nameOffK[chk ? rk3 : 0]; kn1 = g3.nameOffK[chk ? rk3 + 1 : 0];
            sn0 = offS[chk ? srow : 0]; sn1 = offS[chk ? srow + 1 : 0];
        }
        u32 dko = 0, dkt = 0;
#pragma unroll
        for (int w = 0; w < 5; w++) {
            const u32 xk = pk[w];
            dko |= xk ^ po[w];
            dkt |= xk ^ pt[w];
        }
        if (HASH && chk) {
            const u32 len = (u32)(kn1 - kn0);
            if (len != (u32)(sn1 - sn0)) {
                ne = true;
            } else {
                const bool in_lds = lnames && (side_o ? (srow >= rA0 && srow < rA1) : (srow >= rB0 && srow < rB1));
                if (in_lds) {
                    const u32 sb = side_o ? nmb + rnA.skew + (u32)(sn0 - nmA0) : nmb + 16 * rnA.nch + rnB.skew + (u32)(sn0 - nmB0);
                    ne |= !glb_lds_name_eq(g3.nameK, kn0, len, sb);
                } else {
                    ne |= !names_eq(g3.nameK, g3.nameOffK, rk3, side_o ? g.nameA : g.nameB, side_o ? g.nameOffA : g.nameOffB,
                                    srow);
                }
            }
        }
        const bool pa = ik != KD_NONE, pO = io != KD_NONE, pT = itt != KD_NONE;
        const bool a_eq_o = pa == pO && (!pa || dko == 0);
        const bool a_eq_t = pa == pT && (!pa || dkt == 0);
        md = act && a_eq_o;
        cf = act && !a_eq_o && !a_eq_t;
        clean += (act && !a_eq_o && a_eq_t && pO) || (md && pT);
        }
        }
        const u64 bc = __ballot(cf), bm = __ballot(md);
        if (lane == 0) { s_wave[wid] = (u32)__popcll(bc); s_wave[NT / 64 + wid] = (u32)__popcll(bm); }
        __syncthreads();
        u32 pc = 0, pm = 0, nc = 0, nm = 0;
#pragma unroll
        for (int w = 0; w < NT / 64; w++) {
            const u32 xc = s_wave[w], xm = s_wave[NT / 64 + w];
            if (w < wid) { pc += xc; pm += xm; }
            nc += xc;
            nm += xm;
        }
        __syncthreads();
        if (cf) {
            u32* o = sc + 3 * (tc + pc + __builtin_amdgcn_mbcnt_hi((u32)(bc >> 32), __builtin_amdgcn_mbcnt_lo((u32)bc, 0)));
            o[0] = ik; o[1] = io; o[2] = itt;
        }
        if (md) sm[tm + pm + __builtin_amdgcn_mbcnt_hi((u32)(bm >> 32), __builtin_amdgcn_mbcnt_lo((u32)bm, 0))] = make_uint2(io, itt);
        tc += nc;
        tm += nm;
    }
    if (ne) err |= 2u;
    static_assert(2 * IPT < 16, "k_join3b: the clean count's ballot slices");
    {
        const u32 wcl = (u32)__popcll(__ballot(clean & 1)) + 2u * (u32)__popcll(__ballot((clean >> 1) & 1)) +
                        4u * (u32)__popcll(__ballot((clean >> 2) & 1)) + 8u * (u32)__popcll(__ballot((clean >> 3) & 1));
        if (lane == 0) s_wave[2 * (NT / 64) + wid] = wcl;
    }
    __syncthreads();
    u32 tcl = 0;
#pragma unroll
    for (int w = 0; w < NT / 64; w++) tcl += s_wave[2 * (NT / 64) + w];
    if (tid == 0) {
        u32* cc = g.tile_cnt + 4 * tile;
        cc[0] = tcl; cc[1] = tm; cc[2] = 0; cc[3] = tc;
        u64* gs = g.gsum + 2 * (tile / C2_GROUP);
        atomicAdd((unsigned long long*)gs, (unsigned long long)(tc | (u64)tm << 32));
        atomicAdd((unsigned long long*)gs + 1, (unsigned long long)tcl);
    }
    if (!more) break;
    tile = tnext;
    nmA0 = xA0; nmA1 = xA1; nmB0 = xB0; nmB1 = xB1;
    }
    if (err) atomicOr(g.err, err);
}

int merge3_join_device(kd_ctx* ctx, const kd_side& K, const kd_side& O, const kd_side& T, u32* d_conf, uint2* d_md,
                       u64* d_counts, u32* d_err, const u32* ordK, const u32* ordO, const u32* ordT) {
    const u64 nK = K.n, nO = O.n, nT = T.n, total = nO + nT;
    const bool hash = K.key_mode == KD_KEY_HASH;
    const bool perm = ordK || ordO || ordT;
    const bool split = ctx->opt.merge3_split == 1;
    const bool j3_ol = ctx->opt.j3_ol == 1;
    const bool v2 = ctx->opt.j3_v != 0 && !(j3_ol && !perm);
    const int TILE = v2 ? J3B_TILE : J3_TILE;
    if (hash) KD_CHECK((nK == 0 || (K.name && K.name_off)) && (nO == 0 || (O.name && O.name_off)) &&
                       (nT == 0 || (T.name && T.name_off)), "merge3: KD_KEY_HASH needs filenames");
    const u64 ntiles = (total + TILE - 1) / TILE;
    const u64 n_zero = 2 * ((ntiles + C2_GROUP - 1) / C2_GROUP);
    void *part, *apart, *tcnt, *gsum, *gpre, *sconf, *smd, *dz;
    int rc;
    if ((rc = ensure(ctx, "c2.part", (ntiles + 1) * sizeof(u64), &part))) return rc;
    if ((rc = ensure(ctx, "c3.apart", (ntiles + 1) * sizeof(u64), &apart))) return rc;
    if ((rc = ensure(ctx, "c2.tcnt", ntiles * 4 * sizeof(u32), &tcnt))) return rc;
    if ((rc = ensure(ctx, "c2.gsum", n_zero * sizeof(u64), &gsum))) return rc;
    if ((rc = ensure(ctx, "c2.gpre", n_zero * sizeof(u64), &gpre))) return rc;
    if ((rc = ensure(ctx, "c3.sconf", ntiles * C2_STAGE * 12, &sconf))) return rc;
    if ((rc = ensure(ctx, "c3.smd", ntiles * C2_STAGE * sizeof(uint2), &smd))) return rc;
    if ((rc = device_zeros(ctx, &dz))) return rc;
    auto P = [&](const void* p, u64 n) { return n && p ? p : (const void*)dz; };
    const u64* kO = (const u64*)P(O.key, nO);
    const u64* kT = (const u64*)P(T.key, nT);
    const u64* kK = (const u64*)P(K.key, nK);
    rc = launch(ctx, "k_partition2", [&] {
        unsigned nb = (unsigned)((ntiles + C2_PG - 1) / C2_PG);
        if (v2) hipLaunchKernelGGL(k_partition2<J3B_TILE>, dim3(nb), dim3(C2_PNT), 0, ctx->stream, kO, nO, kT, nT, ntiles,
                                   (u64*)part, d_counts, d_err, (u64*)gsum, n_zero);
        else hipLaunchKernelGGL(k_partition2<J3_TILE>, dim3(nb), dim3(C2_PNT), 0, ctx->stream, kO, nO, kT, nT, ntiles,
                                (u64*)part, d_counts, d_err, (u64*)gsum, n_zero);
    });
    if (rc) return rc;
    void* nsplit = nullptr;
    if (v2 && hash && (rc = ensure(ctx, "c3.nsplit", 4 * (ntiles + 1) * sizeof(u64), &nsplit))) return rc;
    rc = launch(ctx, "k_apart3", [&] {
        const u64 lanes = 8 * (ntiles + 1);
        if (v2)
            hipLaunchKernelGGL(k_apart3b, dim3((unsigned)((lanes + 255) / 256)), dim3(256), 0, ctx->stream, kO, nO, kT, nT,
                               (const u64*)part, ntiles, TILE, kK, nK, (u64*)apart, (const u64*)P(O.name_off, nO),
                               (const u64*)P(T.name_off, nT), perm ? J3B_HALO : (u64)0, (u64*)nsplit);
        else
            hipLaunchKernelGGL(k_apart3, dim3((unsigned)((lanes + 255) / 256)), dim3(256), 0, ctx->stream, kO, nO, kT, nT,
                               (const u64*)part, ntiles, TILE, kK, nK, (u64*)apart);
    });
    if (rc) return rc;
    Join3Args a;
    Join2Args& g = a.j;
    g.A = kO; g.oidA = (const u8*)P(O.oid, nO); g.nA = nO;
    g.B = kT; g.oidB = (const u8*)P(T.oid, nT); g.nB = nT;
    g.part = (const u64*)part;
    g.nameA = (const u8*)P(O.name, nO); g.nameOffA = (const u64*)P(O.name_off, nO);
    g.nameB = (const u8*)P(T.name, nT); g.nameOffB = (const u64*)P(T.name_off, nT);
    g.hash_mode = hash ? 1 : 0;
    g.dummy = (const u8*)dz;
    g.ordA = (const u32*)P(ordO, nO); g.ordB = (const u32*)P(ordT, nT);
    g.stage_delta = nullptr;
    g.tile_cnt = (u32*)tcnt; g.gsum = (u64*)gsum; g.err = d_err;
    g.out_delta = g.out_upd = nullptr; g.counts = d_counts;
    g.stage_dkey = g.out_dkey = g.out_ukey = nullptr;
    g.ntiles = ntiles;
    g.walk = ctx->opt.j2_walk;
    a.K = kK; a.oidK = (const u8*)P(K.oid, nK); a.nameK = (const u8*)P(K.name, nK);
    a.nameOffK = (const u64*)P(K.name_off, nK); a.ordK = (const u32*)P(ordK, nK); a.nK = nK;
    a.apart = (const u64*)apart; a.stage_conf = (u32*)sconf; a.stage_md = (uint2*)smd;
    a.nsplit = (const u64*)nsplit;
    void *cand3 = nullptr, *c2 = nullptr;
    if (split) {
        if ((rc = ensure(ctx, "c3.cand3", (total + 1) * 12, &cand3))) return rc;
        if ((rc = ensure(ctx, "c3.c2j", 64, &c2))) return rc;
    }
    auto j3b_grid = [&](const void* kern) {
        if (!J3B_PERSIST) return (unsigned)ntiles;
        return (unsigned)std::max<u64>(1, std::min<u64>(ntiles, (u64)ctx->n_cu * (u64)occupancy(ctx, kern, J3B_NT, 0)));
    };
    rc = launch(ctx, "k_join3", [&] {
#define KD_J3(H, PM, S) hipLaunchKernelGGL((k_join3<C2_NT, J3_IPT, H, PM, S>), dim3((unsigned)ntiles), dim3(C2_NT), 0, ctx->stream, a)
        if (v2) {
#define KD_J3B(H, PM, S) hipLaunchKernelGGL((k_join3b<J3B_NT, J3B_IPT, H, PM, S>), dim3(j3b_grid((const void*)k_join3b<J3B_NT, J3B_IPT, H, PM, S>)), dim3(J3B_NT), 0, ctx->stream, a)
            if (split) {
                if (hash) { if (perm) KD_J3B(true, true, true); else KD_J3B(true, false, true); }
                else { if (perm) KD_J3B(false, true, true); else KD_J3B(false, false, true); }
            } else {
                if (hash) { if (perm) KD_J3B(true, true, false); else KD_J3B(true, false, false); }
                else { if (perm) KD_J3B(false, true, false); else KD_J3B(false, false, false); }
            }
#undef KD_J3B
        } else if (split) {
            if (hash) { if (perm) KD_J3(true, true, true); else KD_J3(true, false, true); }
            else { if (perm) KD_J3(false, true, true); else KD_J3(false, false, true); }
        } else if (j3_ol && !perm) {
            if (hash) hipLaunchKernelGGL((k_join3<C2_NT, J3_IPT, true, false, false, true>), dim3((unsigned)ntiles), dim3(C2_NT), 0, ctx->stream, a);
            else hipLaunchKernelGGL((k_join3<C2_NT, J3_IPT, false, false, false, true>), dim3((unsigned)ntiles), dim3(C2_NT), 0, ctx->stream, a);
        } else {
            if (hash) { if (perm) KD_J3(true, true, false); else KD_J3(true, false, false); }
            else { if (perm) KD_J3(false, true, false); else KD_J3(false, false, false); }
        }
#undef KD_J3
    });
    if (rc) return rc;
    u64* jcounts = split ? (u64*)c2 : d_counts;
    rc = launch(ctx, "k_gscan2", [&] {
        hipLaunchKernelGGL(k_gscan2, dim3(1), dim3(1024), 0, ctx->stream, (const u64*)gsum, (u64)(n_zero / 2),
                           (u64*)gpre, jcounts, 1);
    });
    if (rc) return rc;
    rc = launch(ctx, "k_place3", [&] {
        hipLaunchKernelGGL(k_place3, dim3((unsigned)ntiles), dim3(64), 0, ctx->stream, (const u32*)sconf,
                           (const uint2*)smd, (const u32*)tcnt, (const u64*)gpre, split ? (u32*)cand3 : d_conf, d_md);
    });
    if (rc || !split) return rc;
    return resolve3_have_a(ctx, K, O, T, (const u32*)cand3, (const u64*)c2, d_conf, d_md, d_counts, d_err, ordK, ordO,
                           ordT);
}

int diff2_device(kd_ctx* ctx, const kd_side* A, const kd_side* B, u32 flags, u32* d_delta, u32* d_upd,
                 u64* d_counts, u32* d_err, const u32* ordA, const u32* ordB, u64* d_dkey, u64* d_ukey) {
    Diff2Place pl;
    int rc = diff2_front(ctx, A, B, flags, d_delta, d_upd, d_counts, d_err, ordA, ordB, d_dkey, d_ukey, &pl);
    return rc ? rc : diff2_place(ctx, pl);
}

int diff2_front(kd_ctx* ctx, const kd_side* A, const kd_side* B, u32 flags, u32* d_delta, u32* d_upd, u64* d_counts,
                u32* d_err, const u32* ordA, const u32* ordB, u64* d_dkey, u64* d_ukey, Diff2Place* pl) {
    *pl = Diff2Place{};
    const bool unord = (flags & KD_DIFF_UNORDERED) != 0;
    const u64 nA = A->n, nB = B->n, total = nA + nB;
    KD_CHECK(nA < 0xFFFFFFFFull && nB < 0xFFFFFFFFull, "diff2: side too large for uint32 indices");
    const bool hash = A->key_mode == KD_KEY_HASH || B->key_mode == KD_KEY_HASH;
    KD_CHECK(A->key_mode == B->key_mode, "diff2: key modes differ");
    if (hash) KD_CHECK((nA == 0 || (A->name && A->name_off)) && (nB == 0 || (B->name && B->name_off)),
                       "diff2: KD_KEY_HASH needs filenames");
    const u64 ntiles = (total + C2_TILE - 1) / C2_TILE;
    if (ntiles == 0) {
        KD_HIP(hipMemsetAsync(d_err, 0, sizeof(u32), ctx->stream));
        KD_HIP(hipMemsetAsync(d_counts, 0, 4 * sizeof(u64), ctx->stream));
        return KD_OK;
    }
    void *part, *tcnt = nullptr, *sdel = nullptr, *gsum = nullptr, *gpre = nullptr;
    int rc;
    if ((rc = ensure(ctx, "c2.part", (ntiles + 1) * sizeof(u64), &part))) return rc;
    u64* zero = nullptr;
    u64 n_zero = 0;
    if (!unord) {
        n_zero = 2 * ((ntiles + C2_GROUP - 1) / C2_GROUP);
        if ((rc = ensure(ctx, "c2.tcnt", ntiles * 4 * sizeof(u32), &tcnt))) return rc;
        if ((rc = ensure(ctx, "c2.gsum", n_zero * sizeof(u64), &gsum))) return rc;
        if ((rc = ensure(ctx, "c2.gpre", n_zero * sizeof(u64), &gpre))) return rc;
        if ((rc = ensure(ctx, "c2.sdel", ntiles * C2_STAGE * sizeof(uint2), &sdel))) return rc;
        zero = (u64*)gsum;
    }
    void* skd = nullptr;
    if (d_dkey && !unord && (rc = ensure(ctx, "c2.skd", ntiles * C2_STAGE * sizeof(u64), &skd))) return rc;
    void* dz;
    if ((rc = device_zeros(ctx, &dz))) return rc;
    const u64* kA = nA ? A->key : (const u64*)dz;
    const u64* kB = nB ? B->key : (const u64*)dz;
    const u8* empty_oid = (const u8*)dz;
    rc = launch(ctx, "k_partition2", [&] {
        unsigned nb = (unsigned)((ntiles + C2_PG - 1) / C2_PG);
        hipLaunchKernelGGL(k_partition2<C2_TILE>, dim3(nb), dim3(C2_PNT), 0, ctx->stream, kA, nA, kB, nB, ntiles,
                           (u64*)part, d_counts, d_err, zero, n_zero);
    });
    if (rc) return rc;
    Join2Args g;
    g.A = kA; g.oidA = nA ? A->oid : empty_oid; g.nA = nA;
    g.B = kB; g.oidB = nB ? B->oid : empty_oid; g.nB = nB;
    g.part = (const u64*)part;
    g.nameA = nA && A->name ? A->name : (const u8*)dz;
    g.nameOffA = nA && A->name_off ? A->name_off : (const u64*)dz;
    g.nameB = nB && B->name ? B->name : (const u8*)dz;
    g.nameOffB = nB && B->name_off ? B->name_off : (const u64*)dz;
    g.hash_mode = hash ? 1 : 0;
    g.dummy = (const u8*)dz;
    const bool perm = ordA != nullptr || ordB != nullptr;
    const bool oid_lds = nA + nB >= ctx->opt.j2_oidlds_min;
    const bool j2r = ctx->opt.j2r == 1;
    const int j2r_occ = j2r ? occupancy(ctx, (const void*)k_join2r<C2_NT, C2_IPT>, C2_NT, 0) : 1;
    g.ordA = nA && ordA ? ordA : (const u32*)dz;
    g.ordB = nB && ordB ? ordB : (const u32*)dz;
    g.stage_delta = (uint2*)sdel;
    g.tile_cnt = (u32*)tcnt; g.gsum = (u64*)gsum; g.err = d_err;
    g.out_delta = (uint2*)d_delta; g.out_upd = (uint2*)d_upd; g.counts = d_counts;
    g.stage_dkey = (u64*)skd;
    g.out_dkey = d_dkey; g.out_ukey = d_upd ? d_ukey : nullptr;
    g.ntiles = ntiles;
    g.walk = ctx->opt.j2_walk;
    rc = launch(ctx, "k_join2", [&] {
#define KD_J2(U, H, P) hipLaunchKernelGGL((k_join2<C2_NT, C2_IPT, U, H, P>), dim3((unsigned)ntiles), dim3(C2_NT), 0, ctx->stream, g)
#define KD_J2OL(U) hipLaunchKernelGGL((k_join2<C2_NT, C2_IPT, U, false, false, true>), dim3((unsigned)ntiles), dim3(C2_NT), 0, ctx->stream, g)
#define KD_J2R() hipLaunchKernelGGL((k_join2r<C2_NT, C2_IPT>), dim3((unsigned)std::min<u64>(ntiles, (u64)ctx->n_cu * j2r_occ)), dim3(C2_NT), 0, ctx->stream, g)
        if (perm) {
            if (unord) { if (hash) KD_J2(true, true, true); else KD_J2(true, false, true); }
            else { if (hash) KD_J2(false, true, true); else KD_J2(false, false, true); }
        } else if (!hash && oid_lds) {
            if (unord) KD_J2OL(true);
            else if (j2r) KD_J2R();
            else KD_J2OL(false);
        } else {
            if (unord) { if (hash) KD_J2(true, true, false); else KD_J2(true, false, false); }
            else { if (hash) KD_J2(false, true, false); else KD_J2(false, false, false); }
        }
#undef KD_J2
#undef KD_J2OL
#undef KD_J2R
    });
    if (rc || unord) return rc;
    rc = launch(ctx, "k_gscan2", [&] {
        hipLaunchKernelGGL(k_gscan2, dim3(1), dim3(1024), 0, ctx->stream, (const u64*)gsum, (u64)(n_zero / 2),
                           (u64*)gpre, d_counts, 0);
    });
    if (rc) return rc;
    pl->needed = true;
    pl->ntiles = ntiles;
    pl->sdel = sdel; pl->tcnt = tcnt; pl->gpre = gpre; pl->skd = skd;
    pl->d_delta = d_delta; pl->d_upd = d_upd;
    pl->d_dkey = d_dkey; pl->d_ukey = d_upd ? d_ukey : nullptr;
    return KD_OK;
}

int diff2_place(kd_ctx* ctx, const Diff2Place& pl) {
    if (!pl.needed) return KD_OK;
    return launch(ctx, "k_place2", [&] {
        hipLaunchKernelGGL((k_place2<KD_PLACE_NT>), dim3((unsigned)pl.ntiles), dim3(KD_PLACE_NT), 0, ctx->stream,
                           (const uint2*)pl.sdel, (const u32*)pl.tcnt, (const u64*)pl.gpre, (int)C2_STAGE,
                           (uint2*)pl.d_delta, (uint2*)pl.d_upd, (const u64*)pl.skd, pl.d_dkey, pl.d_ukey);
    });
}

}
```

### kart_amd/csrc/kd_ctx.hip

```cpp
#include <cstdarg>
#include <cstdio>
#include <cstdlib>
#include <cstring>
#include <algorithm>
#include <chrono>
#include <thread>

#include "kd_internal.h"
#include "kd_walkkey.h"

namespace kd {

static thread_local char g_err[1024] = "";

void set_error(const char* fmt, ...) {
    va_list ap;
    va_start(ap, fmt);
    vsnprintf(g_err, sizeof g_err, fmt, ap);
    va_end(ap);
}

constexpr size_t SLAB_BYTES = (size_t)64 << 20, SLAB_PIECE_MAX = (size_t)8 << 20;

int ensure(kd_ctx* ctx, const char* slot, size_t bytes, void** out) {
// ... 137 lines not shown
}

void prof_end(kd_ctx* ctx, const char* name, hipEvent_t a) {
    if (!a) return;
    hipEvent_t b;
    if (ctx->ev_pool.empty()) {
        if (hipEventCreateWithFlags(&b, hipEventDisableSystemFence) != hipSuccess) return;
    } else {
        b = ctx->ev_pool.back();
        ctx->ev_pool.pop_back();
    }
    (void)hipEventRecord(b, ctx->stream);
    ctx->pending.push_back({name, a, b});
}

int prof_flush(kd_ctx* ctx) {
    for (auto& p : ctx->pending) {
        KD_HIP(hipEventSynchronize(p.b));
        float ms = 0;
        KD_HIP(hipEventElapsedTime(&ms, p.a, p.b));
        ProfStat& s = ctx->stats[p.name];
        s.launches++;
        s.ms += ms;
        ctx->ev_pool.push_back(p.a);
        ctx->ev_pool.push_back(p.b);
    }
    ctx->pending.clear();
    return KD_OK;
}

static inline int b64v(u8 c) {
    if (c >= 'A' && c <= 'Z') return c - 'A';
    if (c >= 'a' && c <= 'z') return c - 'a' + 26;
    if (c >= '0' && c <= '9') return c - '0' + 52;
    if (c == '-') return 62;
    if (c == '_') return 63;
    return -1;
}

static inline int int_key(bool neg, u64 mag, u64* key) {
    if (neg ? mag > (1ull << 63) : mag >= (1ull << 63)) return 2;
    *key = wk::int_key(neg ? (i64)(0 - mag) : (i64)mag);
    return 0;
}

static int decode_int_name(const u8* s, int n, u64* key) {
    u8 buf[16];
    int o = 0, acc = 0, bits = 0;
    for (int i = 0; i < n; i++) {
        if (s[i] == '=') break;
        int v = b64v(s[i]);
        if (v < 0) return 1;
        acc = (acc << 6) | v;
        bits += 6;
        if (bits >= 8) {
            bits -= 8;
            if (o >= 16) return 1;
            buf[o++] = (u8)((acc >> bits) & 0xFF);
        }
    }
    if (o < 2 || buf[0] != 0x91) return 1;
    u8 t = buf[1];
    int w = 0;
    bool sgn = false;
    u64 u = 0;
    if (t <= 0x7f) { u = t; }
    else if (t >= 0xe0) { sgn = true; u = (u64)(i64)(int8_t)t; }
    else if (t >= 0xcc && t <= 0xcf) { w = 1 << (t - 0xcc); }
    else if (t >= 0xd0 && t <= 0xd3) { w = 1 << (t - 0xd0); sgn = true; }
    else return 1;
    if (o != 2 + w) return 1;
    if (w) {
        for (int i = 0; i < w; i++) u = (u << 8) | buf[2 + i];
        if (sgn) { int sh = 64 - 8 * w; u = (u64)(((i64)(u << sh)) >> sh); }
    }
    if (sgn) {
        i64 v = (i64)u;
        return int_key(v < 0, v < 0 ? (u64)(-(__int128)v) : (u64)v, key);
    }
    return int_key(false, u, key);
}

template <typename F>
static void par_for(u64 n, F&& f) {
    unsigned nt = std::thread::hardware_concurrency();
    if (nt == 0) nt = 1;
    if (nt > 32) nt = 32;
    if (n < 65536) nt = 1;
    std::vector<std::thread> th;
    u64 chunk = (n + nt - 1) / nt;
    for (unsigned t = 0; t < nt; t++) {
        u64 a = t * chunk, b = std::min<u64>(n, a + chunk);
        if (a >= b) break;
        th.emplace_back([&f, a, b] { for (u64 i = a; i < b; i++) f(i); });
    }
    for (auto& t : th) t.join();
}

static inline u64 fnv1a64(const u8* p, u64 n) {
    u64 h = 1469598103934665603ull;
    for (u64 i = 0; i < n; i++) { h ^= p[i]; h *= 1099511628211ull; }
    return h;
}

}

using namespace kd;

namespace kd {
int occupancy(kd_ctx* ctx, const void* kernel, int block, size_t lds) {
    const auto key = std::make_tuple(kernel, block, lds);
    auto it = ctx->occ.find(key);
    if (it != ctx->occ.end()) return it->second;
    int nb = 0;
    if (hipSetDevice(ctx->device) != hipSuccess ||
        hipOccupancyMaxActiveBlocksPerMultiprocessor(&nb, kernel, block, lds) != hipSuccess || nb <= 0)
        nb = 1;
    ctx->occ[key] = nb;
    return nb;
}
}

extern "C" {

int kd_abi_version(void) { return KD_ABI_VERSION; }

const char* kd_last_error(void) { return kd::g_err; }

__global__ void k_load_probe() {}

namespace {
struct OptDef {
    const char* name;
    const char* env;
    int64_t kd_opts::*i64;
    int kd_opts::*i32;
    uint64_t kd_opts::*u64;
};
const OptDef OPTS[] = {
    {"merge3_join", "KD_MERGE3_JOIN", nullptr, &kd_opts::merge3_join, nullptr},
    {"merge3_split", "KD_MERGE3_SPLIT", nullptr, &kd_opts::merge3_split, nullptr},
    {"j3_ol", "KD_J3_OL", nullptr, &kd_opts::j3_ol, nullptr},
    {"j3_v", "KD_J3_V", nullptr, &kd_opts::j3_v, nullptr},
    {"j2_oidlds_min", "KD_J2_OIDLDS_MIN", nullptr, nullptr, &kd_opts::j2_oidlds_min},
    {"j2r", "KD_J2R", nullptr, &kd_opts::j2r, nullptr},
    {"j2_walk", "KD_J2_WALK", nullptr, &kd_opts::j2_walk, nullptr},
    {"fd_stream", "KD_FD_STREAM", nullptr, &kd_opts::fd_stream, nullptr},
    {"fd_walk", "KD_FD_WALK", nullptr, &kd_opts::fd_walk, nullptr},
    {"pkm_max_blocks", "KD_PKM_MAX_BLOCKS", nullptr, nullptr, &kd_opts::pkm_max_blocks},
    {"trace_host", "KD_TRACE_HOST", nullptr, &kd_opts::trace_host, nullptr},
    {"step_overlap", "KD_STEP_OVERLAP", nullptr, &kd_opts::step_overlap, nullptr},
    {"step_overlap_min", "KD_STEP_OVERLAP_MIN", nullptr, nullptr, &kd_opts::step_overlap_min},
    {"pkm_wave", "KD_PKM_WAVE", nullptr, &kd_opts::pkm_wave, nullptr},
};
void opt_set(kd_opts& o, const OptDef& d, int64_t v) {
    if (d.i32) o.*(d.i32) = (int)v;
    else if (d.u64) o.*(d.u64) = (uint64_t)v;
}
}

int kd_set_option(kd_ctx* ctx, const char* name, int64_t value) {
    KD_CHECK(ctx && name, "kd_set_option: NULL");
    for (const OptDef& d : OPTS)
        if (!strcmp(d.name, name)) {
            opt_set(ctx->opt, d, value);
            return KD_OK;
        }
    KD_CHECK(false, "kd_set_option: unknown option '%s'", name);
}

int kd_get_option(kd_ctx* ctx, const char* name, int64_t* value) {
    KD_CHECK(ctx && name && value, "kd_get_option: NULL");
    for (const OptDef& d : OPTS)
        if (!strcmp(d.name, name)) {
            *value = d.i32 ? (int64_t)(ctx->opt.*(d.i32)) : (int64_t)(ctx->opt.*(d.u64));
            return KD_OK;
        }
    KD_CHECK(false, "kd_get_option: unknown option '%s'", name);
}

int kd_init(int device_ordinal, kd_ctx** out) {
    KD_CHECK(out != nullptr, "kd_init: out is NULL");
    int n = 0;
    KD_HIP(hipGetDeviceCount(&n));
    KD_CHECK(device_ordinal >= 0 && device_ordinal < n, "kd_init: device %d of %d", device_ordinal, n);
    KD_HIP(hipSetDevice(device_ordinal));
    kd_ctx* c = new kd_ctx();
    c->device = device_ordinal;
    for (const OptDef& d : OPTS)
        if (const char* v = std::getenv(d.env)) opt_set(c->opt, d, strtoll(v, nullptr, 10));
    hipError_t e = hipStreamCreateWithFlags(&c->own_stream, hipStreamNonBlocking);
    if (e != hipSuccess) {
        delete c;
        set_error("hipStreamCreate: %s", hipGetErrorString(e));
        return KD_EHIP;
    }
    c->stream = c->own_stream;
    int cu = 0;
    if (hipDeviceGetAttribute(&cu, hipDeviceAttributeMultiprocessorCount, device_ordinal) == hipSuccess && cu > 0)
        c->n_cu = cu;
    {
        void* s = nullptr;
        if (hipMalloc(&s, SLAB_BYTES) == hipSuccess) c->slab = (char*)s;
        c->slab_used = 0;
    }
    for (int j = 0; j < 2; j++) {
        void* h = nullptr;
        if (hipHostMalloc(&h, PIN_CHUNK, hipHostMallocMapped) != hipSuccess) break;
        if (hipEventCreateWithFlags(&c->pin_ev[j], hipEventDisableTiming) != hipSuccess) {
            (void)hipHostFree(h);
            break;
        }
        c->pin[j] = (char*)h;
        void* dp = nullptr;
        if (hipHostGetDevicePointer(&dp, h, 0) == hipSuccess) c->pin_dev[j] = dp;
    }
    hipLaunchKernelGGL(k_load_probe, dim3(1), dim3(64), 0, c->stream);
    if (c->slab) {
        (void)hipMemsetAsync(c->slab, 0, 1024, c->stream);
        (void)hipMemcpyAsync(c->slab + 512, c->slab, 256, hipMemcpyDeviceToDevice, c->stream);
        for (int j = 0; j < 2; j++)
            if (c->pin[j]) {
                std::memset(c->pin[j], 0, PIN_CHUNK);
                (void)hipMemcpyAsync(c->slab + 4096, c->pin[j], PIN_CHUNK, hipMemcpyHostToDevice, c->stream);
                if (c->pin_dev[j])
                    hipLaunchKernelGGL(k_to_host, dim3(64), dim3(256), 0, c->stream, (const u8*)(c->slab + 4096),
                                       (u8*)c->pin_dev[j], (u64)PIN_CHUNK);
                (void)hipEventRecord(c->pin_ev[j], c->stream);
                (void)hipEventSynchronize(c->pin_ev[j]);
            }
        kd_side A{};
        A.n = 1;
        A.key = (const u64*)c->slab;
        A.oid = (const u8*)c->slab;
        A.mem = KD_MEM_DEVICE;
        A.key_mode = KD_KEY_INT;
        u32* out = (u32*)(c->slab + 512);
        c->slab_used = (size_t)8 << 20;
        (void)diff2_device(c, &A, &A, 0, out, out + 8, (u64*)(c->slab + 768), (u32*)(c->slab + 800));
        c->slab_used = 0;
        for (auto& kv : c->bufs)
            if (!kv.second.slab && kv.second.p) (void)hipFree(kv.second.p);
        c->bufs.clear();
    }
    if ((e = hipStreamSynchronize(c->stream)) != hipSuccess) {
        if (c->slab) (void)hipFree(c->slab);
        for (int j = 0; j < 2; j++) {
            if (c->pin[j]) (void)hipHostFree(c->pin[j]);
            if (c->pin_ev[j]) (void)hipEventDestroy(c->pin_ev[j]);
        }
        (void)hipStreamDestroy(c->own_stream);
        delete c;
        set_error("kd_init: %s", hipGetErrorString(e));
        return KD_EHIP;
    }
    *out = c;
    return KD_OK;
}

int kd_fini(kd_ctx* ctx) {
    if (!ctx) return KD_OK;
    (void)hipSetDevice(ctx->device);
    (void)hipStreamSynchronize(ctx->stream);
    prof_flush(ctx);
    comm_release(ctx);
    gather_release(ctx);
    if (ctx->side_stream) {
        (void)hipStreamSynchronize(ctx->side_stream);
        (void)hipStreamDestroy(ctx->side_stream);
    }
    if (ctx->ev_fork) (void)hipEventDestroy(ctx->ev_fork);
    if (ctx->ev_join) (void)hipEventDestroy(ctx->ev_join);
    for (auto& kv : ctx->bufs)
        if (kv.second.p && !kv.second.slab) (void)hipFree(kv.second.p);
    if (ctx->slab) (void)hipFree(ctx->slab);
    for (int j = 0; j < 2; j++) {
        if (ctx->pin[j]) (void)hipHostFree(ctx->pin[j]);
        if (ctx->pin_ev[j]) (void)hipEventDestroy(ctx->pin_ev[j]);
    }
    for (auto e : ctx->ev_pool) (void)hipEventDestroy(e);
    if (ctx->own_stream) (void)hipStreamDestroy(ctx->own_stream);
    delete ctx;
    return KD_OK;
}

int kd_set_stream(kd_ctx* ctx, void* hip_stream) {
    KD_CHECK(ctx, "kd_set_stream: ctx is NULL");
    ctx->stream = hip_stream ? (hipStream_t)hip_stream : ctx->own_stream;
    return KD_OK;
}

int kd_sync(kd_ctx* ctx) {
    KD_CHECK(ctx, "kd_sync: ctx is NULL");
    KD_HIP(hipSetDevice(ctx->device));
    KD_HIP(hipStreamSynchronize(ctx->stream));
    return prof_flush(ctx);
}

void kd_free(void* p) {
    if (!p) return;
    std::free(p);
}

int kd_prof_enable(kd_ctx* ctx, int on) {
    KD_CHECK(ctx, "kd_prof_enable: ctx is NULL");
    ctx->prof = on != 0;
// ... 185 lines not shown
```

### kart_amd/csrc/kd_fielddiff.hip

```cpp
#include <cstdlib>
#include <type_traits>

#include "kd_internal.h"

namespace kd {

typedef const __attribute__((address_space(3))) u32* lp32;
typedef const __attribute__((address_space(1))) u8* gp8;
typedef const __attribute__((address_space(1))) u32* gp32;
typedef const __attribute__((address_space(1))) u32x4* gp128;

enum : u8 { V_NIL = 0, V_INT = 1, V_FLOAT = 2, V_STR = 3, V_BYTES = 4, V_EXT = 5 };

template <class P>
struct DVal {
    u8 cls;
    u8 big;
    i8 ext;
    u64 bits;
    P p;
    u32 len;
};

template <int W, class P>
// ... 906 lines not shown
            a.meta = b.meta = V_NIL;
            a.len = b.len = 0;
            if (so != -2) {
                if ((u32)so >= cvo) return 1;
                seek_value_w(A, po, (u32)so, io, ipo, a);
            }
            if (sn != -2) {
                if ((u32)sn >= cvn) return 1;
                seek_value_w(B, pn, (u32)sn, in, ipn, b);
            }
            r = scalar_eq(a, b);
            if (r == 2) r = payload_eq(a, A, ipo, b, B, ipn, k, q);
        }
        if (r == 1) set_bit<MR>(mk, m, k);
    }
    return 0;
}

template <int M, int G, int S>
__device__ __forceinline__ void coop_differs(const u64 (&a)[M], const u64 (&b)[M], const u32 (&n)[M], bool (&d)[M]) {
    const u32 j = threadIdx.x & (G - 1), grp = (threadIdx.x & 63) / G;
    u32 sa[M], sd[M], nch[M];
    u64 abase[M], ebase[M];
    u32 nmax = 0;
    bool diff[M];
#pragma unroll
    for (int m = 0; m < M; m++) {
        sa[m] = (u32)(a[m] & 15);
        abase[m] = a[m] - sa[m];
        const u64 e = b[m] - sa[m];
        ebase[m] = e & ~(u64)15;
        sd[m] = (u32)(e & 15);
        nch[m] = n[m] ? (n[m] + sa[m] + 15) >> 4 : 0;
        nmax = nch[m] > nmax ? nch[m] : nmax;
        diff[m] = false;
    }
    for (u32 c0 = 0; c0 < nmax; c0 += G * S) {
        u32x4 O[M][S], N0[M][S], N1[M][S];
#pragma unroll
        for (int m = 0; m < M; m++)
#pragma unroll
            for (int s = 0; s < S; s++) {
                const u32 c = c0 + G * s + j;
                const bool act = c < nch[m];
                const u64 oa = abase[m] + 16ull * c, na = ebase[m] + 16ull * c, bend = b[m] + n[m];
                const bool ok0 = act && na < bend && na + 16 > b[m];
                const bool ok1 = act && sd[m] != 0 && na + 16 < bend;
                const u32x4 z = {0, 0, 0, 0};
                O[m][s] = act ? *(gp128)oa : z;
                N0[m][s] = ok0 ? *(gp128)na : z;
                N1[m][s] = ok1 ? *(gp128)(na + 16) : z;
            }
#pragma unroll
        for (int m = 0; m < M; m++)
#pragma unroll
            for (int s = 0; s < S; s++) {
                const u32 c = c0 + G * s + j;
                const u32 q = sd[m] >> 2, sb = sd[m] & 3;
                const u32x4 P0 = N0[m][s], P1 = N1[m][s];
                const bool s1 = q & 1, s2 = q & 2;
                const u32 b0 = s1 ? P0.y : P0.x, b1 = s1 ? P0.z : P0.y, b2 = s1 ? P0.w : P0.z;
                const u32 b3 = s1 ? P1.x : P0.w, b4 = s1 ? P1.y : P1.x, b5 = s1 ? P1.z : P1.y;
                const u32 b6 = s1 ? P1.w : P1.z;
                const u32 t2[5] = {s2 ? b2 : b0, s2 ? b3 : b1, s2 ? b4 : b2, s2 ? b5 : b3, s2 ? b6 : b4};
                const u32 o[4] = {O[m][s].x, O[m][s].y, O[m][s].z, O[m][s].w};
                const int lo = c == 0 ? (int)sa[m] : 0;
                const int hi = (int)n[m] + (int)sa[m] - 16 * (int)c;
                u32 dd = 0;
#pragma unroll
                for (int k = 0; k < 4; k++) {
                    const u32 nw = __builtin_amdgcn_alignbyte(t2[k + 1], t2[k], sb);
                    const u32 lm = lo >= 4 * k + 4 ? 0u : lo <= 4 * k ? ~0u : ~0u << (8 * (lo - 4 * k));
                    const u32 hm = hi <= 4 * k ? 0u : hi >= 4 * k + 4 ? ~0u : (1u << (8 * (hi - 4 * k))) - 1;
                    dd |= (o[k] ^ nw) & lm & hm;
                }
                diff[m] |= c < nch[m] && dd != 0;
            }
    }
#pragma unroll
    for (int m = 0; m < M; m++) d[m] = ((__ballot(diff[m]) >> (G * grp)) & ((1ull << G) - 1)) != 0;
}

template <int M, int G, int S>
__device__ __forceinline__ void coop_differs_u(const u64 (&a)[M], const u64 (&b)[M], const u32 (&n)[M], bool (&d)[M]) {
    const u32 j = threadIdx.x & (G - 1), grp = (threadIdx.x & 63) / G;
    u32 nmax = 0;
    u32 diff[M];
#pragma unroll
    for (int m = 0; m < M; m++) {
        nmax = n[m] > nmax ? n[m] : nmax;
        diff[m] = 0;
    }
    for (u32 c0 = 0; 16 * c0 < nmax; c0 += G * S) {
        u32x4 A[M][S], B[M][S];
#pragma unroll
        for (int m = 0; m < M; m++)
#pragma unroll
            for (int s = 0; s < S; s++) {
                const u32 o = 16 * (c0 + G * s + j);
                const u32 off = min(o, n[m] - 16);
                const u32x4 z = {0, 0, 0, 0};
                A[m][s] = o < n[m] ? *(gp128b)(a[m] + off) : z;
                B[m][s] = o < n[m] ? *(gp128b)(b[m] + off) : z;
            }
#pragma unroll
        for (int m = 0; m < M; m++)
#pragma unroll
            for (int s = 0; s < S; s++) {
                const u32x4 x = A[m][s] ^ B[m][s];
                diff[m] |= x.x | x.y | x.z | x.w;
            }
    }
#pragma unroll
    for (int m = 0; m < M; m++) d[m] = ((__ballot(diff[m] != 0) >> (G * grp)) & ((1ull << G) - 1)) != 0;
}
#ifndef KD_FD_COOPU
#define KD_FD_COOPU 1
#endif
template <int M, int G, int S>
__device__ __forceinline__ void coop_cmp(const u64 (&a)[M], const u64 (&b)[M], const u32 (&n)[M], bool (&d)[M]) {
    if (KD_FD_COOPU) coop_differs_u<M, G, S>(a, b, n, d);
    else coop_differs<M, G, S>(a, b, n, d);
}

constexpr u32 FD_TAB_LDS_MAX = 16384;
#ifndef KD_FD_SHAPE_L
#ifndef KD_FD_TM_L
#define KD_FD_TM_L 3
#endif
#ifndef KD_FD_TGS_L
#define KD_FD_TGS_L 16, 2
#endif
#define KD_FD_SHAPE_L 64, 5, 4, KD_FD_TM_L, KD_FD_TGS_L
#endif
#ifndef KD_FD_SHAPE_S
#define KD_FD_SHAPE_S 32, 8, 3, 1, 16, 2
#endif
template <int UPR, int NH, int NTL, int TM, int TG, int TS>
constexpr int fd_upr(const void*) { return UPR; }
#ifndef KD_FD_SSHAPE
#define KD_FD_SSHAPE 32, 16384
#endif
#ifndef KD_FD_SPF
#define KD_FD_SPF false
#endif
#ifndef KD_FD_STREAM_DEFAULT
#define KD_FD_STREAM_DEFAULT 0
#endif
template <int T, int CAPB>
constexpr int fd_stream_t() { return T; }
typedef __attribute__((address_space(3))) void* fd_lds_vp;
typedef const __attribute__((address_space(1))) void* fd_glb_vp;

#ifdef KD_FD_WPE
#define KD_FD_ATTR __attribute__((amdgpu_waves_per_eu(KD_FD_WPE)))
#else
#define KD_FD_ATTR
#endif
template <int UPR, int NH, int NTL, int TM, int TG, int TS, int MR>
__global__ __launch_bounds__(FD_NT) KD_FD_ATTR void k_fielddiff(const u8* __restrict__ od, const u64* __restrict__ ooff,
                                                     const u8* __restrict__ nd, const u64* __restrict__ noff,
                                                     const uint2* __restrict__ pairs, u64 n_upd_host,
                                                     const u64* __restrict__ n_upd_dev, FdTab tg, FdTabOff to,
                                                     const u8* __restrict__ tab_base,
                                                     u64* __restrict__ masks, u8* __restrict__ status) {
    constexpr int NC = NH + NTL;
    constexpr int LS = 2 * NC;
    constexpr int NCH = (UPR * LS + 63) / 64 * 64;
    constexpr u32 TCAP = UPR;
    static_assert(NTL >= 1, "window shape");
    __shared__ u32x4 s_img[NCH];
    __shared__ u64 s_task[2 * TCAP];
    __shared__ u64 s_res[UPR];
    __shared__ u32 s_ntask;
    extern __shared__ __attribute__((aligned(16))) u8 s_tab[];
    using BL = WBlob<NH, NTL>;
    const int lane = threadIdx.x;
    const bool owner = lane < UPR;
    const bool spec = n_upd_dev && n_upd_host;
    const u64 n_upd = n_upd_dev ? *n_upd_dev : n_upd_host;
    const u64 lim = spec ? n_upd_host : n_upd;
    const u64 end = min(lim, n_upd);
    const u64 step = (u64)gridDim.x * UPR;
    auto load_pair = [&](u64 uu) {
        uint2 p = make_uint2((u32)uu, (u32)uu);
        if (pairs && uu < lim && owner) p = pairs[uu];
        return p;
    };
    auto load_off = [&](uint2 p, bool a, u64& os_, u64& ns_, u32& on_, u32& nn_) {
        os_ = ns_ = 0;
        on_ = nn_ = 0;
        if (a) {
            os_ = ooff[p.x];
            ns_ = noff[p.y];
            on_ = (u32)(ooff[p.x + 1] - os_);
            nn_ = (u32)(noff[p.y + 1] - ns_);
        }
    };
    u64 u0 = (u64)blockIdx.x * UPR;
    if (u0 >= end) return;
    u64 u1 = u0 + step;
    u64 os, ns;
    u32 on, nn;
    load_off(load_pair(u0 + lane), owner && u0 + lane < n_upd, os, ns, on, nn);
    for (u32 i = 16 * lane; i < to.bytes; i += 16 * FD_NT) *(u32x4*)(s_tab + i) = *(gp128)(tab_base + i);
    mp_tab_to_lds();
    if (owner) s_res[lane] = 0;
    if (lane == 0) s_ntask = 0;
    FdTabT<3> tb;
    tb.n_keys = tg.n_keys; tb.words = tg.words; tb.n_lo = tg.n_lo; tb.n_ln = tg.n_ln; tb.maxv = tg.maxv;
    typedef __attribute__((address_space(3))) u8* l8;
    const l8 lt = (l8)s_tab;
    tb.leg_o = (typename ASP<3, u32>::type)(lt + to.leg_o);
    tb.leg_n = (typename ASP<3, u32>::type)(lt + to.leg_n);
    tb.map_o = (typename ASP<3, i16>::type)(lt + to.map_o);
    tb.map_n = (typename ASP<3, i16>::type)(lt + to.map_n);
    tb.cmp = (typename ASP<3, u64>::type)(lt + to.cmp);
    tb.aligned = (typename ASP<3, u8>::type)(lt + to.aligned);
    tb.key_of_val = (typename ASP<3, i16>::type)(lt + to.key_of_val);
    const FdQueue queue{(lds_u64p)s_task, (lds_u32p)&s_ntask, TCAP};
    const u32 img0 = (u32)(size_t)(const __attribute__((address_space(3))) u32x4*)s_img;
    const u64 obase = (u64)od & ~(u64)15, nbase = (u64)nd & ~(u64)15;
    u32 dha = 0, dla = 0, dhb = 0, dlb = 0;
    auto put_desc = [&](u64 os_, u32 an, u64 ns_, u32 bn, bool a) {
        const u64 xa = os_ + ((u64)od & 15), xb = ns_ + ((u64)nd & 15);
        dha = (u32)(xa >> 4);
        dla = a && an ? (u32)((xa + an - 1) >> 4) : 0;
        dhb = (u32)(xb >> 4);
        dlb = a && bn ? (u32)((xb + bn - 1) >> 4) : 0;
        if (!(a && an)) dha = 1;
        if (!(a && bn)) dhb = 1;
    };
    constexpr u32 HALF = (u32)UPR * NC;
    u32 spk[NCH / 64];
#pragma unroll
    for (int k = 0; k < NCH / 64; k++) {
        const u32 c = 64 * k + (lane & 63);
        const bool sb = c >= HALF;
        const u32 cs = sb ? c - HALF : c;
        const u32 ow = cs / NC, i = cs - ow * NC;
        const bool real = ow < (u32)UPR;
        const bool head = i < (u32)NH;
        const u32 off = head ? i : (u32)(NTL - 1) - (i - NH);
        spk[k] = (real ? ow : 0u) | off << 8 | (u32)head << 12 | (u32)real << 13;
    }
    auto stage = [&]() {
#pragma unroll
        for (int k = 0; k < NCH / 64; k++) {
            const u32 c = 64 * k + (lane & 63);
            const bool sb = c >= HALF;
            const int src = (int)(spk[k] & 63);
            const u32 off = (spk[k] >> 8) & 15;
            const bool head = (spk[k] >> 12) & 1, real = (spk[k] >> 13) & 1;
            u32 h, l;
            if (64u * k + 63 < HALF) { h = __shfl(dha, src); l = __shfl(dla, src); }
            else if (64u * k >= HALF) { h = __shfl(dhb, src); l = __shfl(dlb, src); }
            else {
                const u32 ha = __shfl(dha, src), la = __shfl(dla, src), hb_ = __shfl(dhb, src), lb = __shfl(dlb, src);
                h = sb ? hb_ : ha;
                l = sb ? lb : la;
            }
            const u32 ci = head ? h + off : l - off;
            const bool valid = real && (int)(l - h) >= (int)off;
            const u64 addr = (sb ? nbase : obase) + 16ull * ci;
            if (valid) __builtin_amdgcn_global_load_lds((fd_glb_vp)addr, (fd_lds_vp)(s_img + 64 * k), 16, 0, 0);
        }
    };
    put_desc(os, on, ns, nn, owner && u0 + lane < n_upd);
    stage();
    uint2 pr_n = load_pair(u1 + lane);
    __syncthreads();
    for (;;) {
        const u64 u = u0 + lane;
        const bool act = owner && u < n_upd;
        const bool more = u1 < end;
        u64 os_n = 0, ns_n = 0, u2 = end;
        u32 on_n = 0, nn_n = 0;
        if (more) {
            load_off(pr_n, owner && u1 + lane < n_upd, os_n, ns_n, on_n, nn_n);
            u2 = u1 + step;
        }
        u64 mk[4] = {0, 0, 0, 0};
        u8 st = 0;
        u64* m = masks + u * tb.words;
        if (act) {
            for (int w = MR; w < tb.words; w++) m[w] = 0;
            const u64 a0 = (u64)od + os, b0 = (u64)nd + ns;
            BL A, B;
            A.start = a0; A.len = on; A.s0 = (u32)(a0 & 15);
            A.t0 = (int)(((a0 + (on ? on - 1 : 0)) & ~(u64)15) - (a0 & ~(u64)15)) - 16 * (NTL - 1);
            A.img = img0 + 16u * (u32)(lane * NC);
            B.start = b0; B.len = nn; B.s0 = (u32)(b0 & 15);
            B.t0 = (int)(((b0 + (nn ? nn - 1 : 0)) & ~(u64)15) - (b0 & ~(u64)15)) - 16 * (NTL - 1);
            B.img = img0 + 16u * (u32)(UPR * NC + lane * NC);
#if KD_FD_PROBE_NOPARSE
            (void)queue;
#else
            st = KD_FD_HEADF ? diff_one_f<MR>(A, B, tb, mk, m, queue) : diff_one_w<MR>(A, B, tb, mk, m, queue);
#endif
        }
        __syncthreads();
        if (more) {
            put_desc(os_n, on_n, ns_n, nn_n, owner && u1 + lane < n_upd);
            stage();
            pr_n = load_pair(u2 + lane);
        }
#if KD_FD_PROBE_NOCMP
        const u32 nt = 0;
#else
        const u32 nt = min(s_ntask, TCAP);
#endif
        constexpr int M = TM, G = TG, NG = 64 / TG;
        for (u32 t = (u32)lane / G; t < nt; t += NG * M) {
            u64 ta[M], tbb[M], tx[M];
            u32 tn[M];
#pragma unroll
            for (int m = 0; m < M; m++) {
                const u32 tm = t + NG * m;
                const bool h = tm < nt;
                const u64 w0 = h ? s_task[2 * tm] : 0, w1 = h ? s_task[2 * tm + 1] : 0;
                ta[m] = w0 & 0xFFFFFFFFFFFFull;
                tbb[m] = w1 & 0xFFFFFFFFFFFFull;
                tx[m] = w0 >> 48;
                tn[m] = (u32)(w1 >> 48);
            }
            bool d[M];
            coop_cmp<M, G, TS>(ta, tbb, tn, d);
#pragma unroll
            for (int m = 0; m < M; m++)
                if (d[m] && (lane & (G - 1)) == 0) {
                    const u32 ow = (u32)tx[m] & 63, key = (u32)(tx[m] >> 6) & 63;
                    atomicOr((unsigned long long*)&s_res[ow], 1ull << key);
                }
        }
        __syncthreads();
        if (act) {
            mk[0] |= s_res[lane];
            if (st) { mk[0] = mk[1] = mk[2] = mk[3] = 0; }
            store_masks<MR>(m, tb.words, mk, st);
            status[u] = st;
        }
        if (owner) s_res[lane] = 0;
        if (lane == 0) s_ntask = 0;
        if (!more) break;
        __builtin_amdgcn_wave_barrier();
        u0 = u1;
        u1 = u2;
        os = os_n; ns = ns_n; on = on_n; nn = nn_n;
    }
}

template <bool LDS>
struct SBlobT {
    static constexpr bool lds_only = LDS;
    u64 start;
    u32 len;
    u32 s0;
    u32 img;
    __device__ __forceinline__ u32 win(u32 x, u32) const { return LDS ? x : ~0u; }
};

struct FdTile {
    u64 u, co, cn, os, oe, ns, ne;
    u32 nco, ncn;
    bool act;
};

template <int T, u32 CAPC>
__device__ __forceinline__ void fd_load_tile(FdTile& f, u64 tile, u64 n_upd, const u8* od, const u64* ooff, const u8* nd,
                                             const u64* noff) {
    const int lane = threadIdx.x;
    const u64 u0 = tile * T, ue = min(u0 + T, n_upd);
    f.u = u0 + lane;
    f.act = lane < T && f.u < ue;
    const u64 so0 = ooff[u0], so1 = ooff[ue], sn0 = noff[u0], sn1 = noff[ue];
    f.os = f.oe = f.ns = f.ne = 0;
    if (f.act) {
        f.os = ooff[f.u]; f.oe = ooff[f.u + 1];
        f.ns = noff[f.u]; f.ne = noff[f.u + 1];
    }
    f.co = ((u64)od + so0) & ~(u64)15;
    f.cn = ((u64)nd + sn0) & ~(u64)15;
    f.nco = (u32)min<u64>((((u64)od + so1) - f.co + 15) >> 4, CAPC);
    f.ncn = (u32)min<u64>((((u64)nd + sn1) - f.cn + 15) >> 4, CAPC);
}

template <int T, int CAPB, bool PF>
__global__ __launch_bounds__(FD_NT) void k_fielddiff_s(const u8* __restrict__ od, const u64* __restrict__ ooff,
                                                       const u8* __restrict__ nd, const u64* __restrict__ noff,
                                                       u64 n_upd_host, const u64* __restrict__ n_upd_dev,
                                                       FdTab tg, FdTabOff to, const u8* __restrict__ tab_base,
                                                       u64* __restrict__ masks, u8* __restrict__ status) {
    static_assert(T <= FD_NT && CAPB % 512 == 0, "stream shape");
    constexpr u32 CAPC = CAPB / 16;
    constexpr int PL = (int)(2 * CAPC / FD_NT);
    static_assert(!PF || PL * FD_NT == 2 * CAPC, "stream shape");
    __shared__ u32x4 s_img[2 * CAPC + 8];
    __shared__ u32 s_dummy;
    extern __shared__ __attribute__((aligned(16))) u8 s_tab[];
    const int lane = threadIdx.x;
    const u64 n_upd = n_upd_dev ? min(*n_upd_dev, n_upd_host ? n_upd_host : ~0ull) : n_upd_host;
    const u64 ntiles = (n_upd + T - 1) / T;
    if ((u64)blockIdx.x >= ntiles) return;
    for (u32 i = 16 * lane; i < to.bytes; i += 16 * FD_NT) *(u32x4*)(s_tab + i) = *(gp128)(tab_base + i);
    mp_tab_to_lds();
    FdTabT<3> tb;
    tb.n_keys = tg.n_keys; tb.words = tg.words; tb.n_lo = tg.n_lo; tb.n_ln = tg.n_ln; tb.maxv = tg.maxv;
    typedef __attribute__((address_space(3))) u8* l8;
    const l8 lt = (l8)s_tab;
    tb.leg_o = (typename ASP<3, u32>::type)(lt + to.leg_o);
    tb.leg_n = (typename ASP<3, u32>::type)(lt + to.leg_n);
    tb.map_o = (typename ASP<3, i16>::type)(lt + to.map_o);
    tb.map_n = (typename ASP<3, i16>::type)(lt + to.map_n);
    tb.cmp = (typename ASP<3, u64>::type)(lt + to.cmp);
    tb.aligned = (typename ASP<3, u8>::type)(lt + to.aligned);
    tb.key_of_val = (typename ASP<3, i16>::type)(lt + to.key_of_val);
    const FdQueue none{(lds_u64p) nullptr, (lds_u32p)&s_dummy, 0};
    const u32 img_o = (u32)(size_t)(const __attribute__((address_space(3))) u32x4*)s_img;
    const u32 img_n = img_o + 16 * CAPC;
    typedef __attribute__((address_space(3))) u32x4* l128;
    u64 tile = blockIdx.x;
    FdTile cur, nxt;
    fd_load_tile<T, CAPC>(cur, tile, n_upd, od, ooff, nd, noff);
    u32x4 buf[PF ? PL : 1];
    if (PF) {
#pragma unroll
        for (int p = 0; p < PL; p++) {
            const u32 i = 64 * p + lane;
            const bool o = i < cur.nco, n = !o && i < cur.nco + cur.ncn;
            const u64 src = o ? cur.co + 16ull * i : cur.cn + 16ull * (i - cur.nco);
            if (o || n) buf[p] = *(gp128)src;
        }
#pragma unroll
        for (int p = 0; p < PL; p++) {
            const u32 i = 64 * p + lane;
            const bool o = i < cur.nco, n = !o && i < cur.nco + cur.ncn;
            if (o || n) *(l128)(size_t)(o ? img_o + 16 * i : img_n + 16 * (i - cur.nco)) = buf[p];
        }
    }
    u64 nt = tile + gridDim.x;
    if (PF && nt < ntiles) fd_load_tile<T, CAPC>(nxt, nt, n_upd, od, ooff, nd, noff);
    for (;;) {
        const bool more = PF && nt < ntiles;
        if (PF) {
            if (more) {
#pragma unroll
                for (int p = 0; p < PL; p++) {
                    const u32 i = 64 * p + lane;
                    const bool o = i < nxt.nco, n = !o && i < nxt.nco + nxt.ncn;
                    const u64 src = o ? nxt.co + 16ull * i : nxt.cn + 16ull * (i - nxt.nco);
                    if (o || n) buf[p] = *(gp128)src;
                }
            }
        } else {
            for (u32 k = 0; k < cur.nco; k += FD_NT)
                if (k + lane < cur.nco)
                    __builtin_amdgcn_global_load_lds((fd_glb_vp)(cur.co + 16ull * (k + lane)), (fd_lds_vp)(s_img + k), 16, 0, 0);
            for (u32 k = 0; k < cur.ncn; k += FD_NT)
                if (k + lane < cur.ncn)
                    __builtin_amdgcn_global_load_lds((fd_glb_vp)(cur.cn + 16ull * (k + lane)), (fd_lds_vp)(s_img + CAPC + k), 16, 0, 0);
            __syncthreads();
        }
        if (cur.act) {
            SBlobT<true> A, B;
            A.start = (u64)od + cur.os; A.len = (u32)(cur.oe - cur.os); A.s0 = (u32)(A.start & 15);
            A.img = img_o + (u32)((A.start & ~(u64)15) - cur.co);
            B.start = (u64)nd + cur.ns; B.len = (u32)(cur.ne - cur.ns); B.s0 = (u32)(B.start & 15);
            B.img = img_n + (u32)((B.start & ~(u64)15) - cur.cn);
            const bool res = A.start + A.len <= cur.co + 16ull * cur.nco && B.start + B.len <= cur.cn + 16ull * cur.ncn;
            u64* m = masks + cur.u * tb.words;
            for (int w = 4; w < tb.words; w++) m[w] = 0;
            u64 mk[4] = {0, 0, 0, 0};
#if KD_FD_PROBE_NOPARSE
            u8 st = 0;
            (void)none;
            (void)res;
#else
            u8 st;
            if (res) {
                st = diff_one_w(A, B, tb, mk, m, none);
            } else {
                SBlobT<false> GA, GB;
                GA.start = A.start; GA.len = A.len; GA.s0 = A.s0; GA.img = 0;
                GB.start = B.start; GB.len = B.len; GB.s0 = B.s0; GB.img = 0;
                st = diff_one_w(GA, GB, tb, mk, m, none);
            }
#endif
            if (st) { mk[0] = mk[1] = mk[2] = mk[3] = 0; }
            store_masks(m, tb.words, mk, st);
            status[cur.u] = st;
        }
        if (!PF) {
            __syncthreads();
            tile += gridDim.x;
            if (tile >= ntiles) break;
            fd_load_tile<T, CAPC>(cur, tile, n_upd, od, ooff, nd, noff);
            continue;
        }
        if (!more) break;
        const u64 nn = nt + gridDim.x;
        FdTile aft;
        if (nn < ntiles) fd_load_tile<T, CAPC>(aft, nn, n_upd, od, ooff, nd, noff);
#pragma unroll
        for (int p = 0; p < PL; p++) {
            const u32 i = 64 * p + lane;
            const bool o = i < nxt.nco, n = !o && i < nxt.nco + nxt.ncn;
            if (o || n) *(l128)(size_t)(o ? img_o + 16 * i : img_n + 16 * (i - nxt.nco)) = buf[p];
        }
        cur = nxt;
        nt = nn;
        if (nn < ntiles) nxt = aft;
    }
}

#ifndef KD_FDW_SHAPE
#define KD_FDW_SHAPE 1, 16, 2
#endif
#ifndef KD_FDW_CAP
#define KD_FDW_CAP 32
#endif
template <int TM, int TG, int TS>
#ifndef KD_FDW_WPE
#define KD_FDW_WPE 4
#endif
__global__ __launch_bounds__(FD_NT) __attribute__((amdgpu_waves_per_eu(KD_FDW_WPE))) void k_fdwalk(const u8* __restrict__ od, const u64* __restrict__ ooff,
                                                  const u8* __restrict__ nd, const u64* __restrict__ noff,
                                                  const uint2* __restrict__ pairs, u64 n_upd_host,
                                                  const u64* __restrict__ n_upd_dev, u64 n_ent_o, u64 n_ent_n,
                                                  FdTab tg, FdTabOff to, const u8* __restrict__ tab_base,
                                                  u64* __restrict__ masks, u8* __restrict__ status) {
    constexpr u32 TCAP = FD_NT;
    __shared__ u64 s_task[2 * TCAP];
    __shared__ u64 s_res[FD_NT];
    __shared__ u32 s_ntask;
    extern __shared__ __attribute__((aligned(16))) u8 s_tab[];
    const int lane = threadIdx.x;
    const bool spec = n_upd_dev && n_upd_host;
    const u64 n_upd = n_upd_dev ? *n_upd_dev : n_upd_host;
    const u64 lim = spec ? n_upd_host : n_upd;
    const u64 end = min(lim, n_upd);
    const u64 step = (u64)gridDim.x * FD_NT;
    u64 u0 = (u64)blockIdx.x * FD_NT;
    if (u0 >= end) return;
    const u64 olim = (u64)od + ooff[n_ent_o], nlim = (u64)nd + noff[n_ent_n];
    auto load_pair = [&](u64 uu) {
        uint2 p = make_uint2((u32)uu, (u32)uu);
        if (pairs && uu < end) p = pairs[uu];
        return p;
    };
    auto load_off = [&](uint2 p, bool a, u64& os_, u64& ns_, u32& on_, u32& nn_) {
        os_ = ns_ = 0;
        on_ = nn_ = 0;
        if (a) {
            os_ = ooff[p.x];
            ns_ = noff[p.y];
            on_ = (u32)(ooff[p.x + 1] - os_);
            nn_ = (u32)(noff[p.y + 1] - ns_);
        }
    };
    u64 u1 = u0 + step;
    u64 os, ns;
    u32 on, nn;
    load_off(load_pair(u0 + lane), u0 + lane < end, os, ns, on, nn);
    for (u32 i = 16 * lane; i < to.bytes; i += 16 * FD_NT) *(u32x4*)(s_tab + i) = *(gp128)(tab_base + i);
    mp_tab_to_lds();
    s_res[lane] = 0;
    if (lane == 0) s_ntask = 0;
    FdTabT<3> tb;
    tb.n_keys = tg.n_keys; tb.words = tg.words; tb.n_lo = tg.n_lo; tb.n_ln = tg.n_ln; tb.maxv = tg.maxv;
    typedef __attribute__((address_space(3))) u8* l8;
    const l8 lt = (l8)s_tab;
    tb.leg_o = (typename ASP<3, u32>::type)(lt + to.leg_o);
    tb.leg_n = (typename ASP<3, u32>::type)(lt + to.leg_n);
    tb.map_o = (typename ASP<3, i16>::type)(lt + to.map_o);
    tb.map_n = (typename ASP<3, i16>::type)(lt + to.map_n);
    tb.cmp = (typename ASP<3, u64>::type)(lt + to.cmp);
    tb.aligned = (typename ASP<3, u8>::type)(lt + to.aligned);
    tb.key_of_val = (typename ASP<3, i16>::type)(lt + to.key_of_val);
    const FdQueue queue{(lds_u64p)s_task, (lds_u32p)&s_ntask, TCAP};
    uint2 pr_n = load_pair(u1 + lane);
    __syncthreads();
    for (;;) {
        const u64 u = u0 + lane;
        const bool act = u < end;
        const bool more = u1 < end;
        u64 os_n = 0, ns_n = 0, u2 = end;
        u32 on_n = 0, nn_n = 0;
        if (more) {
            load_off(pr_n, u1 + lane < end, os_n, ns_n, on_n, nn_n);
            u2 = u1 + step;
        }
        u64 mk[4] = {0, 0, 0, 0};
        u8 st = 0;
        u64* m = masks + u * tb.words;
        if (act) {
            for (int w = 1; w < tb.words; w++) m[w] = 0;
            const u64 a0 = (u64)od + os, b0 = (u64)nd + ns;
            const HBlobT<true> A{a0, on, a0 + on + 16 > olim, olim}, B{b0, nn, b0 + nn + 16 > nlim, nlim};
            st = diff_one_f<1>(A, B, tb, mk, m, queue);
        }
        __syncthreads();
        if (more) pr_n = load_pair(u2 + lane);
        const u32 nt = min(s_ntask, TCAP);
        constexpr int M = TM, G = TG, NG = 64 / TG;
        for (u32 t = (u32)lane / G; t < nt; t += NG * M) {
            u64 ta[M], tbb[M], tx[M];
            u32 tn[M];
#pragma unroll
            for (int k = 0; k < M; k++) {
                const u32 tm = t + NG * k;
                const bool h = tm < nt;
                const u64 w0 = h ? s_task[2 * tm] : 0, w1 = h ? s_task[2 * tm + 1] : 0;
                ta[k] = w0 & 0xFFFFFFFFFFFFull;
                tbb[k] = w1 & 0xFFFFFFFFFFFFull;
                tx[k] = w0 >> 48;
                tn[k] = (u32)(w1 >> 48);
            }
            bool d[M];
            coop_cmp<M, G, TS>(ta, tbb, tn, d);
#pragma unroll
            for (int k = 0; k < M; k++)
                if (d[k] && (lane & (G - 1)) == 0) {
                    const u32 ow = (u32)tx[k] & 63, key = (u32)(tx[k] >> 6) & 63;
                    atomicOr((unsigned long long*)&s_res[ow], 1ull << key);
                }
        }
        __syncthreads();
        if (act) {
            mk[0] |= s_res[lane];
            if (st) { mk[0] = mk[1] = mk[2] = mk[3] = 0; }
            store_masks<1>(m, tb.words, mk, st);
            status[u] = st;
        }
        s_res[lane] = 0;
        if (lane == 0) s_ntask = 0;
        if (!more) break;
        __builtin_amdgcn_wave_barrier();
        u0 = u1;
        u1 = u2;
        os = os_n; ns = ns_n; on = on_n; nn = nn_n;
    }
}

__global__ __launch_bounds__(FD_NT) void k_fielddiff_g(const u8* __restrict__ od, const u64* __restrict__ ooff,
                                                       const u8* __restrict__ nd, const u64* __restrict__ noff,
                                                       const uint2* __restrict__ pairs, u64 n_upd_host,
                                                       const u64* __restrict__ n_upd_dev, FdTab tb,
                                                       u64* __restrict__ masks, u8* __restrict__ status) {
    const int lane = threadIdx.x;
    const bool spec = n_upd_dev && n_upd_host;
    const u64 n_upd = n_upd_dev ? *n_upd_dev : n_upd_host;
    const u64 lim = spec ? n_upd_host : n_upd;
    for (u64 u0 = (u64)blockIdx.x * FD_NT; u0 < lim; u0 += (u64)gridDim.x * FD_NT) {
        const u64 u = u0 + lane;
        uint2 pr = make_uint2((u32)u, (u32)u);
        if (pairs && u < lim) pr = pairs[u];
        if (u0 >= n_upd || u >= n_upd) break;
        const u64 os = ooff[pr.x], ns = noff[pr.y];
        const u32 on = (u32)(ooff[pr.x + 1] - os);
        const u32 nn = (u32)(noff[pr.y + 1] - ns);
        u64* m = masks + u * tb.words;
        for (int w = 4; w < tb.words; w++) m[w] = 0;
        u64 mk[4] = {0, 0, 0, 0};
        const u8 st = diff_one((gp8)(od + os), on, (gp8)(nd + ns), nn, tb, mk, m);
        if (st) { mk[0] = mk[1] = mk[2] = mk[3] = 0; }
        store_masks(m, tb.words, mk, st);
        status[u] = st;
    }
}

}

using namespace kd;

extern "C" int kd_fielddiff(kd_ctx* ctx, const kd_blobs* ob, const kd_blobs* nb, const uint32_t* pu, uint64_t n_upd,
                            const uint64_t* d_n_upd, uint32_t pairs_mem, const kd_legend_maps* mp, uint64_t* masks,
                            uint8_t* status, uint32_t out_mem) {
    KD_CHECK(ctx && ob && nb && mp && masks && status, "kd_fielddiff: NULL argument");
    KD_CHECK(mp->n_keys >= 0 && mp->words == (mp->n_keys + 63) / 64 && mp->words >= 1, "kd_fielddiff: bad words");
    KD_CHECK(mp->n_leg_old > 0 && mp->n_leg_new > 0 && mp->n_leg_old <= 4096 && mp->n_leg_new <= 4096,
             "kd_fielddiff: bad legend counts");
    KD_CHECK(d_n_upd == nullptr || out_mem == KD_MEM_DEVICE, "kd_fielddiff: device count needs device outputs");
    KD_HIP(hipSetDevice(ctx->device));
    int rc;
    const int nk = mp->n_keys, nlo = mp->n_leg_old, nln = mp->n_leg_new, W = mp->words;
    int maxv = 1;
    std::vector<u32> nvo(nlo, 0);
    for (int l = 0; l < nlo; l++)
        for (int k = 0; k < nk; k++) {
            int s = mp->map_old[(size_t)l * nk + k];
            if (s >= 0 && (u32)s + 1 > nvo[l]) nvo[l] = (u32)s + 1;
        }
    for (int l = 0; l < nlo; l++) maxv = std::max<int>(maxv, (int)nvo[l]);
    std::vector<u8> aligned((size_t)nlo * nln, 0);
    for (int a = 0; a < nlo; a++)
        for (int b = 0; b < nln; b++) {
            bool ok = true;
            for (int k = 0; k < nk && ok; k++) {
                if (!((mp->cmp_mask[k >> 6] >> (k & 63)) & 1)) continue;
                int so = mp->map_old[(size_t)a * nk + k], sn = mp->map_new[(size_t)b * nk + k];
                ok = so == sn && so != -1;
            }
            aligned[(size_t)a * nln + b] = ok ? 1 : 0;
        }
    std::vector<i16> kov((size_t)nlo * maxv, -1);
    for (int l = 0; l < nlo; l++)
        for (int k = 0; k < nk; k++) {
            if (!((mp->cmp_mask[k >> 6] >> (k & 63)) & 1)) continue;
            int s = mp->map_old[(size_t)l * nk + k];
            if (s >= 0 && s < maxv) kov[(size_t)l * maxv + s] = (i16)k;
        }
    auto al = [](size_t x) { return (x + 15) & ~(size_t)15; };
    size_t o_lo = 0, o_ln = al(o_lo + (size_t)nlo * 40), o_mo = al(o_ln + (size_t)nln * 40),
           o_mn = al(o_mo + (size_t)nlo * nk * 2), o_cmp = al(o_mn + (size_t)nln * nk * 2),
           o_al = al(o_cmp + (size_t)W * 8), o_kov = al(o_al + aligned.size()), o_nv = al(o_kov + kov.size() * 2),
           o_end = al(o_nv + (size_t)nlo * 4);
    std::vector<u8> h(o_end, 0);
    std::memcpy(&h[o_lo], mp->leg_old_hex, (size_t)nlo * 40);
    std::memcpy(&h[o_ln], mp->leg_new_hex, (size_t)nln * 40);
    std::memcpy(&h[o_mo], mp->map_old, (size_t)nlo * nk * 2);
    std::memcpy(&h[o_mn], mp->map_new, (size_t)nln * nk * 2);
    std::memcpy(&h[o_cmp], mp->cmp_mask, (size_t)W * 8);
    std::memcpy(&h[o_al], aligned.data(), aligned.size());
    if (!kov.empty()) std::memcpy(&h[o_kov], kov.data(), kov.size() * 2);
    std::memcpy(&h[o_nv], nvo.data(), (size_t)nlo * 4);
    void* dt;
    if ((rc = ensure(ctx, "fd.tab", o_end, &dt))) return rc;
    if (ctx->fd_tab != h) {
        ctx->fd_tab.swap(h);
        KD_HIP(hipMemcpyAsync(dt, ctx->fd_tab.data(), o_end, hipMemcpyHostToDevice, ctx->stream));
    }
    FdTab tb;
    tb.n_keys = nk; tb.words = W; tb.n_lo = nlo; tb.n_ln = nln; tb.maxv = maxv;
    const u8* base = (const u8*)dt;
    tb.leg_o = (const u32*)(base + o_lo); tb.leg_n = (const u32*)(base + o_ln);
    tb.map_o = (const i16*)(base + o_mo); tb.map_n = (const i16*)(base + o_mn);
    tb.cmp = (const u64*)(base + o_cmp); tb.aligned = base + o_al;
    tb.key_of_val = (const i16*)(base + o_kov);

    const void *d_od, *d_ooff, *d_nd, *d_noff, *d_pu = nullptr;
    u64 ob_bytes = 0, nb_bytes = 0;
    if (ob->mem == KD_MEM_HOST) ob_bytes = ob->off[ob->n];
    if (nb->mem == KD_MEM_HOST) nb_bytes = nb->off[nb->n];
    if ((rc = stage_in(ctx, "fd.ooff", ob->off, (ob->n + 1) * 8, ob->mem, &d_ooff))) return rc;
    if ((rc = stage_in(ctx, "fd.od", ob->data, ob_bytes ? ob_bytes : 1, ob->mem, &d_od))) return rc;
    if ((rc = stage_in(ctx, "fd.noff", nb->off, (nb->n + 1) * 8, nb->mem, &d_noff))) return rc;
    if ((rc = stage_in(ctx, "fd.nd", nb->data, nb_bytes ? nb_bytes : 1, nb->mem, &d_nd))) return rc;
    if (d_n_upd) {
        KD_CHECK(pu == nullptr || pairs_mem == KD_MEM_DEVICE, "kd_fielddiff: device count needs device pairs");
        d_pu = pu;
    } else if (pu && n_upd) {
        if ((rc = stage_in(ctx, "fd.pu", pu, n_upd * 8, pairs_mem, &d_pu))) return rc;
    }
    u64 *d_masks = masks;
    u8* d_status = status;
    if (out_mem == KD_MEM_HOST && n_upd && !d_n_upd) {
        void *a, *b;
        if ((rc = ensure(ctx, "fd.masks", n_upd * W * 8, &a))) return rc;
        if ((rc = ensure(ctx, "fd.status", n_upd, &b))) return rc;
        d_masks = (u64*)a;
        d_status = (u8*)b;
    }
    if (n_upd == 0 && d_n_upd == nullptr) return KD_OK;
    u64 work = d_n_upd ? (n_upd ? n_upd : (u64)1 << 22) : n_upd;
    auto typical = [](const kd_blobs* b) -> u64 {
        if (b->size_hint) return b->size_hint;
        if (b->mem == KD_MEM_HOST && b->n) return (b->off[b->n] - b->off[0] + b->n - 1) / b->n;
        return 256;
    };
    const u64 typ = std::max(typical(ob), typical(nb));
    FdTabOff to;
    to.leg_o = (u32)o_lo; to.leg_n = (u32)o_ln; to.map_o = (u32)o_mo; to.map_n = (u32)o_mn; to.cmp = (u32)o_cmp;
    to.aligned = (u32)o_al; to.key_of_val = (u32)o_kov; to.bytes = (u32)o_end;
    const bool lds_tab = o_end <= FD_TAB_LDS_MAX;
    const bool small = typ <= 144;
    const int stream_env = ctx->opt.fd_stream;
    const bool stream = lds_tab && d_pu == nullptr && (stream_env >= 0 ? stream_env > 0 : !small && KD_FD_STREAM_DEFAULT);
    const int walk_env = ctx->opt.fd_walk;
    const bool walk = lds_tab && !stream && walk_env > 0;
    const void* kern = walk ? (const void*)k_fdwalk<KD_FDW_SHAPE>
                       : stream ? (const void*)k_fielddiff_s<KD_FD_SSHAPE, KD_FD_SPF>
                       : !lds_tab ? (const void*)k_fielddiff_g
                       : small ? (W == 1 ? (const void*)k_fielddiff<KD_FD_SHAPE_S, 1> : (const void*)k_fielddiff<KD_FD_SHAPE_S, 4>)
                       : (W == 1 ? (const void*)k_fielddiff<KD_FD_SHAPE_L, 1> : (const void*)k_fielddiff<KD_FD_SHAPE_L, 4>);
    int per_cu = 0;
    KD_HIP(hipOccupancyMaxActiveBlocksPerMultiprocessor(&per_cu, kern, FD_NT, lds_tab ? o_end : 0));
#ifndef KD_FD_CAP
#define KD_FD_CAP 12
#endif
    per_cu = std::max(1, std::min(per_cu, walk ? KD_FDW_CAP : stream ? 16 : KD_FD_CAP));
    const u64 upr = walk ? (u64)FD_NT : stream ? (u64)fd_stream_t<KD_FD_SSHAPE>() : !lds_tab ? FD_NT : small ? fd_upr<KD_FD_SHAPE_S>(nullptr) : fd_upr<KD_FD_SHAPE_L>(nullptr);
    unsigned blocks = (unsigned)std::min<u64>((work + upr - 1) / upr, (u64)ctx->n_cu * (u64)per_cu);
    if (blocks == 0) blocks = 1;
    rc = launch(ctx, "k_fielddiff", [&] {
        auto args = [&](auto kern) {
            hipLaunchKernelGGL(kern, dim3(blocks), dim3(FD_NT), o_end, ctx->stream, (const u8*)d_od, (const u64*)d_ooff,
                               (const u8*)d_nd, (const u64*)d_noff, (const uint2*)d_pu, n_upd, d_n_upd,
                               tb, to, (const u8*)dt, d_masks, d_status);
        };
        if (walk)
            hipLaunchKernelGGL((k_fdwalk<KD_FDW_SHAPE>), dim3(blocks), dim3(FD_NT), o_end, ctx->stream, (const u8*)d_od,
                               (const u64*)d_ooff, (const u8*)d_nd, (const u64*)d_noff, (const uint2*)d_pu, n_upd, d_n_upd,
                               (u64)ob->n, (u64)nb->n, tb, to, (const u8*)dt, d_masks, d_status);
        else if (stream)
            hipLaunchKernelGGL((k_fielddiff_s<KD_FD_SSHAPE, KD_FD_SPF>), dim3(blocks), dim3(FD_NT), o_end, ctx->stream, (const u8*)d_od,
                               (const u64*)d_ooff, (const u8*)d_nd, (const u64*)d_noff, n_upd, d_n_upd, tb, to,
                               (const u8*)dt, d_masks, d_status);
        else if (!lds_tab)
            hipLaunchKernelGGL(k_fielddiff_g, dim3(blocks), dim3(FD_NT), 0, ctx->stream, (const u8*)d_od, (const u64*)d_ooff,
                               (const u8*)d_nd, (const u64*)d_noff, (const uint2*)d_pu, n_upd, d_n_upd, tb, d_masks,
                               d_status);
        else if (small) W == 1 ? args(k_fielddiff<KD_FD_SHAPE_S, 1>) : args(k_fielddiff<KD_FD_SHAPE_S, 4>);
        else W == 1 ? args(k_fielddiff<KD_FD_SHAPE_L, 1>) : args(k_fielddiff<KD_FD_SHAPE_L, 4>);
    });
    if (rc) return rc;
    if (out_mem == KD_MEM_HOST) {
        if ((rc = stage_d2h(ctx, masks, d_masks, n_upd * W * 8)) || (rc = stage_d2h(ctx, status, d_status, n_upd))) return rc;
        prof_flush(ctx);
    }
    return KD_OK;
}
```

### kart_amd/csrc/kd_internal.h

```cpp
#pragma once
#include <hip/hip_runtime.h>

#include <cstdint>
#include <cstring>
#include <map>
#include <utility>
#include <mutex>
#include <string>
#include <tuple>
#include <vector>

#include "kartdiff.h"

typedef uint8_t u8;
typedef uint16_t u16;
typedef uint32_t u32;
typedef uint64_t u64;
typedef int64_t i64;
typedef int16_t i16;
typedef int8_t i8;
typedef unsigned u32x4 __attribute__((ext_vector_type(4)));
typedef uint64_t u64x2 __attribute__((ext_vector_type(2)));

namespace kd {

void set_error(const char* fmt, ...);

#define KD_HIP(call)                                                                        \
    do {                                                                                    \
        hipError_t e_ = (call);                                                             \
        if (e_ != hipSuccess) {                                                             \
            ::kd::set_error("%s:%d %s: %s", __FILE__, __LINE__, #call, hipGetErrorString(e_)); \
            return KD_EHIP;                                                                 \
        }                                                                                   \
    } while (0)

#define KD_CHECK(cond, ...)            \
    do {                               \
        if (!(cond)) {                 \
            ::kd::set_error(__VA_ARGS__); \
            return KD_EINVAL;          \
        }                              \
    } while (0)

struct DevBuf {
    void* p = nullptr;
    size_t bytes = 0;
    bool slab = false;
};

struct ProfStat {
    u64 launches = 0;
    double ms = 0;
};

struct PendingEv {
    std::string name;
    hipEvent_t a, b;
};

}

struct kd_opts {
    int merge3_join = 1;
    int merge3_split = 0;
    int j3_ol = 0;
    int j3_v = 1;
    uint64_t j2_oidlds_min = 1ull << 26;
    int j2r = 0;
    int j2_walk = 1;
    int fd_stream = -1;
    int fd_walk = -1;
    uint64_t pkm_max_blocks = 1ull << 26;
    int trace_host = 0;
    int step_overlap = 1;
    uint64_t step_overlap_min = 1ull << 26;
    int pkm_wave = -1;
};

struct kd_ctx {
    int device = 0;
    kd_opts opt;
    hipStream_t own_stream = nullptr;
    hipStream_t stream = nullptr;
    std::map<std::string, kd::DevBuf> bufs;
    hipStream_t side_stream = nullptr;
    hipEvent_t ev_fork = nullptr, ev_join = nullptr;
    hipStream_t step_main = nullptr;
    bool prof = false;
    std::string prof_only;
    std::vector<hipEvent_t> ev_pool;
    std::vector<kd::PendingEv> pending;
    std::map<std::string, kd::ProfStat> stats;
    std::vector<uint8_t> fd_tab;
    int n_cu = 256;
    void* comm = nullptr;
    int nranks = 1, rank = 0;
    std::vector<int> group_devs;
    std::vector<void*> group_comms;
    hipStream_t comm_stream = nullptr;
    hipEvent_t ev_counts = nullptr, ev_gathered = nullptr;
    uint64_t* h_counts_pin = nullptr;
    int h_counts_ranks = 0;
    uint64_t gather_send_cap = 0;
    int occ_resolve3 = 0;
    std::map<std::tuple<const void*, int, size_t>, int> occ;
    uint32_t rs_epoch = 0;
    int pkm_cur = 0;
    void* pkm_zero_ptr[2] = {nullptr, nullptr};
    uint64_t pkm_zero_nb[2] = {0, 0};
    char* slab = nullptr;
    size_t slab_used = 0;
    char* pin[2] = {nullptr, nullptr};
    void* pin_dev[2] = {nullptr, nullptr};
    hipEvent_t pin_ev[2] = {nullptr, nullptr};
    int pin_next = 0;
};

namespace kd {

void gather_release(kd_ctx* ctx);
int ensure(kd_ctx* ctx, const char* slot, size_t bytes, void** out);
int stage_h2d(kd_ctx* ctx, void* dst, const void* src, size_t bytes);
void host_mark(kd_ctx* ctx, const char* name);
int stage_d2h(kd_ctx* ctx, void* dst, const void* src, size_t bytes);

int device_zeros(kd_ctx* ctx, void** out);

int occupancy(kd_ctx* ctx, const void* kernel, int block, size_t lds);

struct StreamScope {
    kd_ctx* ctx;
    hipStream_t saved;
    StreamScope(kd_ctx* c, hipStream_t s) : ctx(c), saved(c->stream) {
        c->step_main = saved;
        c->stream = s;
    }
    ~StreamScope() {
        ctx->stream = saved;
        ctx->step_main = nullptr;
    }
    StreamScope(const StreamScope&) = delete;
    StreamScope& operator=(const StreamScope&) = delete;
};

void prof_begin(kd_ctx* ctx, const char* name, hipEvent_t* a);
void prof_end(kd_ctx* ctx, const char* name, hipEvent_t a);
int prof_flush(kd_ctx* ctx);

inline bool prof_on(const kd_ctx* ctx, const char* name) {
    return ctx->prof && (ctx->prof_only.empty() || ctx->prof_only.find("," + std::string(name) + ",") != std::string::npos);
}

template <typename F>
inline int launch(kd_ctx* ctx, const char* name, F&& f) {
    hipEvent_t a = nullptr;
    const bool prof = prof_on(ctx, name);
    if (prof) prof_begin(ctx, name, &a);
    f();
    hipError_t e = hipGetLastError();
    if (prof) prof_end(ctx, name, a);
    if (e != hipSuccess) {
        set_error("launch %s: %s", name, hipGetErrorString(e));
        return KD_EHIP;
    }
    return KD_OK;
}

int stage_in(kd_ctx* ctx, const char* slot, const void* p, size_t bytes, u32 mem, const void** dev);
int stage_side(kd_ctx* ctx, const kd_side* s, const char* tag, kd_side* dev);
int check_side(const kd_side* s, const char* which);
void comm_release(kd_ctx* ctx);

int resolve3_have_a(kd_ctx* ctx, const kd_side& K, const kd_side& O, const kd_side& T, const u32* cand3, const u64* c2,
                    u32* d_conf, uint2* d_md, u64* d_counts, u32* d_err, const u32* ordK, const u32* ordO,
                    const u32* ordT);
int merge3_join_device(kd_ctx* ctx, const kd_side& K, const kd_side& O, const kd_side& T, u32* d_conf, uint2* d_md,
                       u64* d_counts, u32* d_err, const u32* ordK = nullptr, const u32* ordO = nullptr,
                       const u32* ordT = nullptr);
int diff2_device(kd_ctx* ctx, const kd_side* A, const kd_side* B, u32 flags, u32* d_delta,
                 u32* d_upd, u64* d_counts, u32* d_err, const u32* ordA = nullptr, const u32* ordB = nullptr,
                 u64* d_dkey = nullptr, u64* d_ukey = nullptr);
struct Diff2Place {
    bool needed = false;
    u64 ntiles = 0;
    const void *sdel = nullptr, *tcnt = nullptr, *gpre = nullptr, *skd = nullptr;
    u32 *d_delta = nullptr, *d_upd = nullptr;
    u64 *d_dkey = nullptr, *d_ukey = nullptr;
};
int diff2_front(kd_ctx* ctx, const kd_side* A, const kd_side* B, u32 flags, u32* d_delta, u32* d_upd, u64* d_counts,
                u32* d_err, const u32* ordA, const u32* ordB, u64* d_dkey, u64* d_ukey, Diff2Place* pl);
int diff2_place(kd_ctx* ctx, const Diff2Place& pl);
int delta_pk_order(kd_ctx* ctx, const kd_side* base, const kd_side* target, const u32* d_delta, const u64* d_keys,
                   u64 cap, const u64* d_n, i64 pk_lo, i64 pk_hi, i64* d_pk, u32* d_perm, bool lds_free);
#ifndef KD_C2_NT
#define KD_C2_NT 256
#endif
constexpr int C2_NT = KD_C2_NT;
#ifndef KD_C2_IPT
#define KD_C2_IPT 4
#endif
constexpr int C2_IPT = KD_C2_IPT;
constexpr int C2_TILE = C2_NT * C2_IPT;

}
```

Measured before the change: 36240 M feature-pairs/s.

## Move group scan to side stream; field diff reads partitioned update counters

The join kernel now also accumulates per-tile update counts into 64 strided partial counters. The single-block group scan that used to run on the main stream before the field diff can then move onto the side stream, alongside placement and pk ordering. The field-diff kernels sum those partials with a wave reduction instead of waiting for the scanned count, which takes the serial scan off the critical path. In exchange the join adds an extra atomic per tile, and an LDS-free 64-lane scan variant is added so the side-stream scan does not compete with the field diff for LDS.

```diff
diff --git a/kart_amd/csrc/kd_classify.hip b/kart_amd/csrc/kd_classify.hip
--- a/kart_amd/csrc/kd_classify.hip
+++ b/kart_amd/csrc/kd_classify.hip
@@ -408,7 +408,7 @@
     int rc;
     if ((rc = ensure(ctx, "c2.part", (ntiles + 1) * 8, &p))) return rc;
     if ((rc = ensure(ctx, "c2.tcnt", ntiles * 16, &p))) return rc;
-    if ((rc = ensure(ctx, "c2.gsum", 2 * (ntiles / 64 + 1) * 8, &p))) return rc;
+    if ((rc = ensure(ctx, "c2.gsum", (2 * (ntiles / 64 + 1) + C2_UCNT * C2_UCNT_STRIDE) * 8, &p))) return rc;
     if ((rc = ensure(ctx, "c2.sdel", ntiles * (C2_TILE + 64) * 8, &p))) return rc;
     (void)max_updates;
     return KD_OK;
@@ -475,15 +475,22 @@
     if ((rc = device_zeros(ctx, &dz))) return rc;
     const u32* oa = s->base_order ? (s->base->n ? s->base_order : (const u32*)dz) : nullptr;
     const u32* ob = s->target_order ? (s->target->n ? s->target_order : (const u32*)dz) : nullptr;
+    const int ov = ctx->opt.step_overlap;
+    const bool place_aside = !(have_fd && s->d_pairs);
+    const bool placed = !(s->flags & KD_DIFF_UNORDERED) && s->base->n + s->target->n > 0;
+    const bool overlap = ov > 0 && have_fd && placed && (place_aside || have_dpk || have_upk) &&
+                         s->base->n + s->target->n >= ctx->opt.step_overlap_min;
+    const bool scan_aside = overlap && place_aside && ctx->opt.step_count > 0;
     Diff2Place pl;
     if ((rc = diff2_front(ctx, s->base, s->target, s->flags, s->d_delta, s->d_upd, s->d_counts, s->d_err, oa, ob,
-                          s->d_delta_key, s->d_upd_key, &pl)))
+                          s->d_delta_key, s->d_upd_key, &pl, scan_aside)))
         return rc;
-    const int ov = ctx->opt.step_overlap;
+    if (!scan_aside && (rc = diff2_scan(ctx, pl, false))) return rc;
     auto field_diff = [&]() -> int {
-        return have_fd ? kd_fielddiff(ctx, s->old_blobs, s->new_blobs, s->d_pairs, s->upd_cap, s->d_counts + 1,
-                                      KD_MEM_DEVICE, s->maps, s->d_masks, s->d_status, KD_MEM_DEVICE)
-                       : KD_OK;
+        if (!have_fd) return KD_OK;
+        return fielddiff_device(ctx, s->old_blobs, s->new_blobs, s->d_pairs, s->upd_cap,
+                                scan_aside ? pl.ucnt : s->d_counts + 1, scan_aside ? (int)C2_UCNT : 0, KD_MEM_DEVICE,
+                                s->maps, s->d_masks, s->d_status, KD_MEM_DEVICE);
     };
     auto pk_orders = [&](bool lds_free) -> int {
         int r = KD_OK;
@@ -495,9 +502,6 @@
                                s->pk_hi, s->d_upd_pk, s->d_upd_perm, lds_free);
         return r;
     };
-    const bool place_aside = !(have_fd && s->d_pairs);
-    const bool overlap = ov > 0 && have_fd && pl.needed && (place_aside || have_dpk || have_upk) &&
-                         s->base->n + s->target->n >= ctx->opt.step_overlap_min;
     const int wave = ctx->opt.pkm_wave;
     if (!overlap) {
         if ((rc = diff2_place(ctx, pl)) || (rc = field_diff())) return rc;
@@ -514,7 +518,8 @@
     auto side_work = [&]() -> int {
         StreamScope scope(ctx, side);
         KD_HIP(hipStreamWaitEvent(side, ctx->ev_fork, 0));
-        int r = place_aside ? diff2_place(ctx, pl) : KD_OK;
+        int r = scan_aside ? diff2_scan(ctx, pl, true) : KD_OK;
+        if (!r && place_aside) r = diff2_place(ctx, pl);
         return r ? r : pk_orders(wave != 0);
     };
     int rc_fd, rc_side = KD_OK;
diff --git a/kart_amd/csrc/kd_classify2.hip b/kart_amd/csrc/kd_classify2.hip
--- a/kart_amd/csrc/kd_classify2.hip
+++ b/kart_amd/csrc/kd_classify2.hip
@@ -115,6 +115,7 @@
     uint2* stage_delta;
     u32* tile_cnt;
     u64* gsum;
+    u64* ucnt;
     uint2* out_delta;
     uint2* out_upd;
     u64* stage_dkey;
@@ -498,6 +499,14 @@
     }
 }
 
+__device__ __forceinline__ void tile_sums(const Join2Args& g, u64 tile, const TileCounts& c) {
+    const int tid = threadIdx.x;
+    if (tid > 2) return;
+    u64* p = tid < 2 ? g.gsum + 2 * (tile / C2_GROUP) + tid : g.ucnt ? g.ucnt + (tile % C2_UCNT) * C2_UCNT_STRIDE : nullptr;
+    const u64 v = tid == 0 ? c.tnd | (u64)c.tnu << 32 : tid == 1 ? (c.tnd - c.tnu - c.tdel) | (u64)c.tdel << 32 : c.tnu;
+    if (tid < 2 || (g.ucnt && v)) atomicAdd((unsigned long long*)p, (unsigned long long)v);
+}
+
 template <int NT, int IPT, bool UNORD, bool HASH, bool PERM, bool OL = false>
 __global__ __launch_bounds__(NT) void k_join2(Join2Args g) {
     using LD = Join2Lds<NT, IPT>;
@@ -645,15 +654,12 @@
     tile_write<IPT>(rec, c, q.i0, q.j0, sd, su, sA, sB, kd, ku);
     if (!UNORD && tid == 0) {
         u32* cc = g.tile_cnt + 4 * tile;
-        const u32 tins = c.tnd - c.tnu - c.tdel;
-        cc[0] = tins;
+        cc[0] = c.tnd - c.tnu - c.tdel;
         cc[1] = c.tnu;
         cc[2] = c.tdel;
         cc[3] = c.tnd;
-        u64* gs = g.gsum + 2 * (tile / C2_GROUP);
-        atomicAdd((unsigned long long*)gs, (unsigned long long)(c.tnd | (u64)c.tnu << 32));
-        atomicAdd((unsigned long long*)gs + 1, (unsigned long long)(tins | (u64)c.tdel << 32));
-    }
+    }
+    if (!UNORD) tile_sums(g, tile, c);
 }
 
 template <int NT, int IPT>
@@ -766,10 +772,8 @@
             cc[1] = c.tnu;
             cc[2] = c.tdel;
             cc[3] = c.tnd;
-            u64* gs = g.gsum + 2 * (tile / C2_GROUP);
-            atomicAdd((unsigned long long*)gs, (unsigned long long)(c.tnd | (u64)c.tnu << 32));
-            atomicAdd((unsigned long long*)gs + 1, (unsigned long long)(tins | (u64)c.tdel << 32));
-        }
+        }
+        tile_sums(g, tile, c);
         if (!more) break;
         lds_barrier();
         deposit(nxt);
@@ -832,6 +836,43 @@
         counts[1] = layout ? cd : cu;
         counts[2] = layout ? cu : cx;
         counts[3] = layout ? 0 : cd;
+    }
+}
+
+__global__ __launch_bounds__(64) void k_gscan2w(const u64* __restrict__ gsum, u64 ngroups, u64* __restrict__ gpre,
+                                                u64* __restrict__ counts) {
+    const int lane = threadIdx.x;
+    const u32x4* g4 = (const u32x4*)gsum;
+    u32x4* p4 = (u32x4*)gpre;
+    const u64 per = (ngroups + 63) / 64;
+    const u64 k0 = (u64)lane * per, k1 = k0 + per < ngroups ? k0 + per : ngroups;
+    u64 td = 0, tu = 0, ti = 0, tx = 0;
+#pragma unroll 8
+    for (u64 k = k0; k < k1; k++) {
+        const u32x4 v = g4[k];
+        td += v.x; tu += v.y; ti += v.z; tx += v.w;
+    }
+    u64 sd = td, su = tu;
+#pragma unroll
+    for (int o = 1; o < 64; o <<= 1) {
+        const u64 yd = __shfl_up(sd, o, 64), yu = __shfl_up(su, o, 64);
+        if (lane >= o) { sd += yd; su += yu; }
+    }
+#pragma unroll
+    for (int o = 32; o > 0; o >>= 1) { ti += __shfl_xor(ti, o, 64); tx += __shfl_xor(tx, o, 64); }
+    u64 pd = sd - td, pu = su - tu;
+#pragma unroll 8
+    for (u64 k = k0; k < k1; k++) {
+        const u32x4 v = g4[k];
+        p4[k] = u32x4{(u32)pd, (u32)(pd >> 32), (u32)pu, (u32)(pu >> 32)};
+        pd += v.x;
+        pu += v.y;
+    }
+    if (lane == 63) {
+        counts[0] = ti;
+        counts[1] = su;
+        counts[2] = tx;
+        counts[3] = sd;
     }
 }
 
@@ -1717,7 +1758,7 @@
     g.dummy = (const u8*)dz;
     g.ordA = (const u32*)P(ordO, nO); g.ordB = (const u32*)P(ordT, nT);
     g.stage_delta = nullptr;
-    g.tile_cnt = (u32*)tcnt; g.gsum = (u64*)gsum; g.err = d_err;
+    g.tile_cnt = (u32*)tcnt; g.gsum = (u64*)gsum; g.ucnt = nullptr; g.err = d_err;
     g.out_delta = g.out_upd = nullptr; g.counts = d_counts;
     g.stage_dkey = g.out_dkey = g.out_ukey = nullptr;
     g.ntiles = ntiles;
@@ -1778,12 +1819,13 @@
 int diff2_device(kd_ctx* ctx, const kd_side* A, const kd_side* B, u32 flags, u32* d_delta, u32* d_upd,
                  u64* d_counts, u32* d_err, const u32* ordA, const u32* ordB, u64* d_dkey, u64* d_ukey) {
     Diff2Place pl;
-    int rc = diff2_front(ctx, A, B, flags, d_delta, d_upd, d_counts, d_err, ordA, ordB, d_dkey, d_ukey, &pl);
+    int rc = diff2_front(ctx, A, B, flags, d_delta, d_upd, d_counts, d_err, ordA, ordB, d_dkey, d_ukey, &pl, false);
+    if (!rc) rc = diff2_scan(ctx, pl, false);
     return rc ? rc : diff2_place(ctx, pl);
 }
 
 int diff2_front(kd_ctx* ctx, const kd_side* A, const kd_side* B, u32 flags, u32* d_delta, u32* d_upd, u64* d_counts,
-                u32* d_err, const u32* ordA, const u32* ordB, u64* d_dkey, u64* d_ukey, Diff2Place* pl) {
+                u32* d_err, const u32* ordA, const u32* ordB, u64* d_dkey, u64* d_ukey, Diff2Place* pl, bool count_upd) {
     *pl = Diff2Place{};
     const bool unord = (flags & KD_DIFF_UNORDERED) != 0;
     const u64 nA = A->n, nB = B->n, total = nA + nB;
@@ -1806,11 +1848,12 @@
     if (!unord) {
         n_zero = 2 * ((ntiles + C2_GROUP - 1) / C2_GROUP);
         if ((rc = ensure(ctx, "c2.tcnt", ntiles * 4 * sizeof(u32), &tcnt))) return rc;
-        if ((rc = ensure(ctx, "c2.gsum", n_zero * sizeof(u64), &gsum))) return rc;
+        if ((rc = ensure(ctx, "c2.gsum", (n_zero + C2_UCNT * C2_UCNT_STRIDE) * sizeof(u64), &gsum))) return rc;
         if ((rc = ensure(ctx, "c2.gpre", n_zero * sizeof(u64), &gpre))) return rc;
         if ((rc = ensure(ctx, "c2.sdel", ntiles * C2_STAGE * sizeof(uint2), &sdel))) return rc;
         zero = (u64*)gsum;
     }
+    u64* ucnt = !unord && count_upd ? (u64*)gsum + n_zero : nullptr;
     void* skd = nullptr;
     if (d_dkey && !unord && (rc = ensure(ctx, "c2.skd", ntiles * C2_STAGE * sizeof(u64), &skd))) return rc;
     void* dz;
@@ -1821,7 +1864,7 @@
     rc = launch(ctx, "k_partition2", [&] {
         unsigned nb = (unsigned)((ntiles + C2_PG - 1) / C2_PG);
         hipLaunchKernelGGL(k_partition2<C2_TILE>, dim3(nb), dim3(C2_PNT), 0, ctx->stream, kA, nA, kB, nB, ntiles,
-                           (u64*)part, d_counts, d_err, zero, n_zero);
+                           (u64*)part, d_counts, d_err, zero, n_zero + (ucnt ? C2_UCNT * C2_UCNT_STRIDE : 0));
     });
     if (rc) return rc;
     Join2Args g;
@@ -1841,7 +1884,7 @@
     g.ordA = nA && ordA ? ordA : (const u32*)dz;
     g.ordB = nB && ordB ? ordB : (const u32*)dz;
     g.stage_delta = (uint2*)sdel;
-    g.tile_cnt = (u32*)tcnt; g.gsum = (u64*)gsum; g.err = d_err;
+    g.tile_cnt = (u32*)tcnt; g.gsum = (u64*)gsum; g.ucnt = ucnt; g.err = d_err;
     g.out_delta = (uint2*)d_delta; g.out_upd = (uint2*)d_upd; g.counts = d_counts;
     g.stage_dkey = (u64*)skd;
     g.out_dkey = d_dkey; g.out_ukey = d_upd ? d_ukey : nullptr;
@@ -1867,17 +1910,27 @@
 #undef KD_J2R
     });
     if (rc || unord) return rc;
-    rc = launch(ctx, "k_gscan2", [&] {
-        hipLaunchKernelGGL(k_gscan2, dim3(1), dim3(1024), 0, ctx->stream, (const u64*)gsum, (u64)(n_zero / 2),
-                           (u64*)gpre, d_counts, 0);
-    });
-    if (rc) return rc;
     pl->needed = true;
     pl->ntiles = ntiles;
-    pl->sdel = sdel; pl->tcnt = tcnt; pl->gpre = gpre; pl->skd = skd;
+    pl->sdel = sdel; pl->tcnt = tcnt; pl->gsum = gsum; pl->gpre = gpre; pl->skd = skd;
+    pl->ucnt = ucnt;
+    pl->d_counts = d_counts;
     pl->d_delta = d_delta; pl->d_upd = d_upd;
     pl->d_dkey = d_dkey; pl->d_ukey = d_upd ? d_ukey : nullptr;
     return KD_OK;
+}
+
+int diff2_scan(kd_ctx* ctx, const Diff2Place& pl, bool lds_free) {
+    if (!pl.needed) return KD_OK;
+    const u64 ngroups = (pl.ntiles + C2_GROUP - 1) / C2_GROUP;
+    return launch(ctx, "k_gscan2", [&] {
+        if (lds_free)
+            hipLaunchKernelGGL(k_gscan2w, dim3(1), dim3(64), 0, ctx->stream, (const u64*)pl.gsum, ngroups, (u64*)pl.gpre,
+                               pl.d_counts);
+        else
+            hipLaunchKernelGGL(k_gscan2, dim3(1), dim3(1024), 0, ctx->stream, (const u64*)pl.gsum, ngroups, (u64*)pl.gpre,
+                               pl.d_counts, 0);
+    });
 }
 
 int diff2_place(kd_ctx* ctx, const Diff2Place& pl) {
diff --git a/kart_amd/csrc/kd_ctx.hip b/kart_amd/csrc/kd_ctx.hip
--- a/kart_amd/csrc/kd_ctx.hip
+++ b/kart_amd/csrc/kd_ctx.hip
@@ -313,6 +313,7 @@
     {"step_overlap", "KD_STEP_OVERLAP", nullptr, &kd_opts::step_overlap, nullptr},
     {"step_overlap_min", "KD_STEP_OVERLAP_MIN", nullptr, nullptr, &kd_opts::step_overlap_min},
     {"pkm_wave", "KD_PKM_WAVE", nullptr, &kd_opts::pkm_wave, nullptr},
+    {"step_count", "KD_STEP_COUNT", nullptr, &kd_opts::step_count, nullptr},
 };
 void opt_set(kd_opts& o, const OptDef& d, int64_t v) {
     if (d.i32) o.*(d.i32) = (int)v;
diff --git a/kart_amd/csrc/kd_fielddiff.hip b/kart_amd/csrc/kd_fielddiff.hip
--- a/kart_amd/csrc/kd_fielddiff.hip
+++ b/kart_amd/csrc/kd_fielddiff.hip
@@ -1082,6 +1082,16 @@
 typedef __attribute__((address_space(3))) void* fd_lds_vp;
 typedef const __attribute__((address_space(1))) void* fd_glb_vp;
 
+__device__ __forceinline__ u64 fd_dev_count(const u64* __restrict__ p, int n_part) {
+    if (n_part <= 0) return *p;
+    const int lane = threadIdx.x & 63;
+    u64 v = lane < n_part ? p[(size_t)lane * C2_UCNT_STRIDE] : 0;
+#pragma unroll
+    for (int o = 32; o > 0; o >>= 1) v += __shfl_xor(v, o, 64);
+    const u32 lo = __builtin_amdgcn_readfirstlane((u32)v), hi = __builtin_amdgcn_readfirstlane((u32)(v >> 32));
+    return (u64)hi << 32 | lo;
+}
+
 #ifdef KD_FD_WPE
 #define KD_FD_ATTR __attribute__((amdgpu_waves_per_eu(KD_FD_WPE)))
 #else
@@ -1091,7 +1101,7 @@
 __global__ __launch_bounds__(FD_NT) KD_FD_ATTR void k_fielddiff(const u8* __restrict__ od, const u64* __restrict__ ooff,
                                                      const u8* __restrict__ nd, const u64* __restrict__ noff,
                                                      const uint2* __restrict__ pairs, u64 n_upd_host,
-                                                     const u64* __restrict__ n_upd_dev, FdTab tg, FdTabOff to,
+                                                     const u64* __restrict__ n_upd_dev, int n_part, FdTab tg, FdTabOff to,
                                                      const u8* __restrict__ tab_base,
                                                      u64* __restrict__ masks, u8* __restrict__ status) {
     constexpr int NC = NH + NTL;
@@ -1108,7 +1118,7 @@
     const int lane = threadIdx.x;
     const bool owner = lane < UPR;
     const bool spec = n_upd_dev && n_upd_host;
-    const u64 n_upd = n_upd_dev ? *n_upd_dev : n_upd_host;
+    const u64 n_upd = n_upd_dev ? fd_dev_count(n_upd_dev, n_part) : n_upd_host;
     const u64 lim = spec ? n_upd_host : n_upd;
     const u64 end = min(lim, n_upd);
     const u64 step = (u64)gridDim.x * UPR;
@@ -1318,7 +1328,7 @@
 template <int T, int CAPB, bool PF>
 __global__ __launch_bounds__(FD_NT) void k_fielddiff_s(const u8* __restrict__ od, const u64* __restrict__ ooff,
                                                        const u8* __restrict__ nd, const u64* __restrict__ noff,
-                                                       u64 n_upd_host, const u64* __restrict__ n_upd_dev,
+                                                       u64 n_upd_host, const u64* __restrict__ n_upd_dev, int n_part,
                                                        FdTab tg, FdTabOff to, const u8* __restrict__ tab_base,
                                                        u64* __restrict__ masks, u8* __restrict__ status) {
     static_assert(T <= FD_NT && CAPB % 512 == 0, "stream shape");
@@ -1329,7 +1339,7 @@
     __shared__ u32 s_dummy;
     extern __shared__ __attribute__((aligned(16))) u8 s_tab[];
     const int lane = threadIdx.x;
-    const u64 n_upd = n_upd_dev ? min(*n_upd_dev, n_upd_host ? n_upd_host : ~0ull) : n_upd_host;
+    const u64 n_upd = n_upd_dev ? min(fd_dev_count(n_upd_dev, n_part), n_upd_host ? n_upd_host : ~0ull) : n_upd_host;
     const u64 ntiles = (n_upd + T - 1) / T;
     if ((u64)blockIdx.x >= ntiles) return;
     for (u32 i = 16 * lane; i < to.bytes; i += 16 * FD_NT) *(u32x4*)(s_tab + i) = *(gp128)(tab_base + i);
@@ -1456,7 +1466,7 @@
 __global__ __launch_bounds__(FD_NT) __attribute__((amdgpu_waves_per_eu(KD_FDW_WPE))) void k_fdwalk(const u8* __restrict__ od, const u64* __restrict__ ooff,
                                                   const u8* __restrict__ nd, const u64* __restrict__ noff,
                                                   const uint2* __restrict__ pairs, u64 n_upd_host,
-                                                  const u64* __restrict__ n_upd_dev, u64 n_ent_o, u64 n_ent_n,
+                                                  const u64* __restrict__ n_upd_dev, int n_part, u64 n_ent_o, u64 n_ent_n,
                                                   FdTab tg, FdTabOff to, const u8* __restrict__ tab_base,
                                                   u64* __restrict__ masks, u8* __restrict__ status) {
     constexpr u32 TCAP = FD_NT;
@@ -1466,7 +1476,7 @@
     extern __shared__ __attribute__((aligned(16))) u8 s_tab[];
     const int lane = threadIdx.x;
     const bool spec = n_upd_dev && n_upd_host;
-    const u64 n_upd = n_upd_dev ? *n_upd_dev : n_upd_host;
+    const u64 n_upd = n_upd_dev ? fd_dev_count(n_upd_dev, n_part) : n_upd_host;
     const u64 lim = spec ? n_upd_host : n_upd;
     const u64 end = min(lim, n_upd);
     const u64 step = (u64)gridDim.x * FD_NT;
@@ -1575,11 +1585,11 @@
 __global__ __launch_bounds__(FD_NT) void k_fielddiff_g(const u8* __restrict__ od, const u64* __restrict__ ooff,
                                                        const u8* __restrict__ nd, const u64* __restrict__ noff,
                                                        const uint2* __restrict__ pairs, u64 n_upd_host,
-                                                       const u64* __restrict__ n_upd_dev, FdTab tb,
+                                                       const u64* __restrict__ n_upd_dev, int n_part, FdTab tb,
                                                        u64* __restrict__ masks, u8* __restrict__ status) {
     const int lane = threadIdx.x;
     const bool spec = n_upd_dev && n_upd_host;
-    const u64 n_upd = n_upd_dev ? *n_upd_dev : n_upd_host;
+    const u64 n_upd = n_upd_dev ? fd_dev_count(n_upd_dev, n_part) : n_upd_host;
     const u64 lim = spec ? n_upd_host : n_upd;
     for (u64 u0 = (u64)blockIdx.x * FD_NT; u0 < lim; u0 += (u64)gridDim.x * FD_NT) {
         const u64 u = u0 + lane;
@@ -1599,18 +1609,15 @@
     }
 }
 
-}
-
-using namespace kd;
-
-extern "C" int kd_fielddiff(kd_ctx* ctx, const kd_blobs* ob, const kd_blobs* nb, const uint32_t* pu, uint64_t n_upd,
-                            const uint64_t* d_n_upd, uint32_t pairs_mem, const kd_legend_maps* mp, uint64_t* masks,
-                            uint8_t* status, uint32_t out_mem) {
+int fielddiff_device(kd_ctx* ctx, const kd_blobs* ob, const kd_blobs* nb, const uint32_t* pu, uint64_t n_upd,
+                     const uint64_t* d_n_upd, int n_part, uint32_t pairs_mem, const kd_legend_maps* mp, uint64_t* masks,
+                     uint8_t* status, uint32_t out_mem) {
     KD_CHECK(ctx && ob && nb && mp && masks && status, "kd_fielddiff: NULL argument");
     KD_CHECK(mp->n_keys >= 0 && mp->words == (mp->n_keys + 63) / 64 && mp->words >= 1, "kd_fielddiff: bad words");
     KD_CHECK(mp->n_leg_old > 0 && mp->n_leg_new > 0 && mp->n_leg_old <= 4096 && mp->n_leg_new <= 4096,
              "kd_fielddiff: bad legend counts");
     KD_CHECK(d_n_upd == nullptr || out_mem == KD_MEM_DEVICE, "kd_fielddiff: device count needs device outputs");
+    KD_CHECK(n_part >= 0 && n_part <= 64 && (n_part == 0 || d_n_upd), "kd_fielddiff: bad partial counters");
     KD_HIP(hipSetDevice(ctx->device));
     int rc;
     const int nk = mp->n_keys, nlo = mp->n_leg_old, nln = mp->n_leg_new, W = mp->words;
@@ -1725,20 +1732,20 @@
     rc = launch(ctx, "k_fielddiff", [&] {
         auto args = [&](auto kern) {
             hipLaunchKernelGGL(kern, dim3(blocks), dim3(FD_NT), o_end, ctx->stream, (const u8*)d_od, (const u64*)d_ooff,
-                               (const u8*)d_nd, (const u64*)d_noff, (const uint2*)d_pu, n_upd, d_n_upd,
+                               (const u8*)d_nd, (const u64*)d_noff, (const uint2*)d_pu, n_upd, d_n_upd, n_part,
                                tb, to, (const u8*)dt, d_masks, d_status);
         };
         if (walk)
             hipLaunchKernelGGL((k_fdwalk<KD_FDW_SHAPE>), dim3(blocks), dim3(FD_NT), o_end, ctx->stream, (const u8*)d_od,
-                               (const u64*)d_ooff, (const u8*)d_nd, (const u64*)d_noff, (const uint2*)d_pu, n_upd, d_n_upd,
+                               (const u64*)d_ooff, (const u8*)d_nd, (const u64*)d_noff, (const uint2*)d_pu, n_upd, d_n_upd, n_part,
                                (u64)ob->n, (u64)nb->n, tb, to, (const u8*)dt, d_masks, d_status);
         else if (stream)
             hipLaunchKernelGGL((k_fielddiff_s<KD_FD_SSHAPE, KD_FD_SPF>), dim3(blocks), dim3(FD_NT), o_end, ctx->stream, (const u8*)d_od,
-                               (const u64*)d_ooff, (const u8*)d_nd, (const u64*)d_noff, n_upd, d_n_upd, tb, to,
+                               (const u64*)d_ooff, (const u8*)d_nd, (const u64*)d_noff, n_upd, d_n_upd, n_part, tb, to,
                                (const u8*)dt, d_masks, d_status);
         else if (!lds_tab)
             hipLaunchKernelGGL(k_fielddiff_g, dim3(blocks), dim3(FD_NT), 0, ctx->stream, (const u8*)d_od, (const u64*)d_ooff,
-                               (const u8*)d_nd, (const u64*)d_noff, (const uint2*)d_pu, n_upd, d_n_upd, tb, d_masks,
+                               (const u8*)d_nd, (const u64*)d_noff, (const uint2*)d_pu, n_upd, d_n_upd, n_part, tb, d_masks,
                                d_status);
         else if (small) W == 1 ? args(k_fielddiff<KD_FD_SHAPE_S, 1>) : args(k_fielddiff<KD_FD_SHAPE_S, 4>);
         else W == 1 ? args(k_fielddiff<KD_FD_SHAPE_L, 1>) : args(k_fielddiff<KD_FD_SHAPE_L, 4>);
@@ -1750,3 +1757,11 @@
     }
     return KD_OK;
 }
+
+}
+
+extern "C" int kd_fielddiff(kd_ctx* ctx, const kd_blobs* ob, const kd_blobs* nb, const uint32_t* pu, uint64_t n_upd,
+                            const uint64_t* d_n_upd, uint32_t pairs_mem, const kd_legend_maps* mp, uint64_t* masks,
+                            uint8_t* status, uint32_t out_mem) {
+    return kd::fielddiff_device(ctx, ob, nb, pu, n_upd, d_n_upd, 0, pairs_mem, mp, masks, status, out_mem);
+}
diff --git a/kart_amd/csrc/kd_internal.h b/kart_amd/csrc/kd_internal.h
--- a/kart_amd/csrc/kd_internal.h
+++ b/kart_amd/csrc/kd_internal.h
@@ -58,6 +58,10 @@
     std::string name;
     hipEvent_t a, b;
 };
+
+int fielddiff_device(kd_ctx* ctx, const kd_blobs* ob, const kd_blobs* nb, const uint32_t* pu, uint64_t n_upd,
+                     const uint64_t* d_n_upd, int n_part, uint32_t pairs_mem, const kd_legend_maps* mp, uint64_t* masks,
+                     uint8_t* status, uint32_t out_mem);
 
 }
 
@@ -75,6 +79,7 @@
     int trace_host = 0;
     int step_overlap = 1;
     uint64_t step_overlap_min = 1ull << 26;
+    int step_count = 1;
     int pkm_wave = -1;
 };
 
@@ -181,15 +186,19 @@
 int diff2_device(kd_ctx* ctx, const kd_side* A, const kd_side* B, u32 flags, u32* d_delta,
                  u32* d_upd, u64* d_counts, u32* d_err, const u32* ordA = nullptr, const u32* ordB = nullptr,
                  u64* d_dkey = nullptr, u64* d_ukey = nullptr);
+constexpr u64 C2_UCNT = 64, C2_UCNT_STRIDE = 16;
 struct Diff2Place {
     bool needed = false;
     u64 ntiles = 0;
-    const void *sdel = nullptr, *tcnt = nullptr, *gpre = nullptr, *skd = nullptr;
+    const void *sdel = nullptr, *tcnt = nullptr, *gsum = nullptr, *gpre = nullptr, *skd = nullptr;
+    const u64* ucnt = nullptr;
+    u64* d_counts = nullptr;
     u32 *d_delta = nullptr, *d_upd = nullptr;
     u64 *d_dkey = nullptr, *d_ukey = nullptr;
 };
 int diff2_front(kd_ctx* ctx, const kd_side* A, const kd_side* B, u32 flags, u32* d_delta, u32* d_upd, u64* d_counts,
-                u32* d_err, const u32* ordA, const u32* ordB, u64* d_dkey, u64* d_ukey, Diff2Place* pl);
+                u32* d_err, const u32* ordA, const u32* ordB, u64* d_dkey, u64* d_ukey, Diff2Place* pl, bool count_upd);
+int diff2_scan(kd_ctx* ctx, const Diff2Place& pl, bool lds_free);
 int diff2_place(kd_ctx* ctx, const Diff2Place& pl);
 int delta_pk_order(kd_ctx* ctx, const kd_side* base, const kd_side* target, const u32* d_delta, const u64* d_keys,
                    u64 cap, const u64* d_n, i64 pk_lo, i64 pk_hi, i64* d_pk, u32* d_perm, bool lds_free);
```

Measured after the change: 37210 M feature-pairs/s, median of 6. 1.03x the previous value.
